# HuiyangYu/TGSFilter

Measured on AMD Instinct MI355X. Metric: filtered Gbases/sec (end-to-end, excl. gzip I/O), higher is better.
Workload: dtype u8

## Files before the change

### tgsfilter_amd/csrc/tgsf_emul_rt.h

```cpp
#pragma once
#include "tgsf_emul.h"
typedef void* rt_stream;
typedef void* rt_event;
static int rt_set_device(int) { return 0; }
static int rt_malloc(void** p, size_t n) { *p = calloc(n ? n : 1, 1); return *p ? 0 : 1; }
static void rt_free(void* p) { free(p); }
static void rt_host_free(void*) {}
static int rt_memset(void* p, int v, size_t n, rt_stream) { memset(p, v, n); return 0; }
static int rt_h2d(void* d, const void* s, size_t n, rt_stream) { memcpy(d, s, n); return 0; }
static int rt_d2h(void* d, const void* s, size_t n, rt_stream) { memcpy(d, s, n); return 0; }
static int rt_stream_create(rt_stream* s) { *s = nullptr; return 0; }
static void rt_stream_destroy(rt_stream) {}
static int rt_sync(rt_stream) { return 0; }
static int rt_device_sync() { return 0; }
static int rt_stream_wait(rt_stream, rt_event) { return 0; }
static int rt_event_create(rt_event* e) { *e = nullptr; return 0; }
static void rt_event_destroy(rt_event) {}
static int rt_event_record(rt_event, rt_stream) { return 0; }
static int rt_event_sync(rt_event) { return 0; }
static int rt_event_ms(float* ms, rt_event, rt_event) { *ms = 0.0f; return 0; }
static int rt_last_error() { return 0; }
static const char* rt_errstr(int) { return "emulation error"; }
template <class F>
static void emul_launch(unsigned grid, unsigned block, F f)
{
    using namespace tgsf_emul;
    gridDim = {grid, 1, 1}; blockDim = {block, 1, 1};
    const char* ord = getenv("TGSF_EMUL_ORDER");
    const bool reverse = ord && !strcmp(ord, "reverse");
    for (unsigned b0 = 0; b0 < grid; b0++)
        for (unsigned t0 = 0; t0 < block; t0++) {
            const unsigned b = reverse ? grid - 1 - b0 : b0, t = reverse ? block - 1 - t0 : t0;
            blockIdx = {b, 0, 0}; threadIdx = {t, 0, 0}; f();
        }
}
#define TGSF_LAUNCH(kernel, grid, block, stream, ...) ((void)(stream), emul_launch((grid), (block), [&] { kernel(__VA_ARGS__); }))
#define TGSF_LAUNCH_COOP(kernel, grid, block, stream, ...) ((void)(stream), emul_launch((grid), 1u, [&] { kernel(__VA_ARGS__); }))
static unsigned grid_cap(unsigned g) { return g > 8u ? 8u : g; }
```

### tgsfilter_amd/csrc/tgsf_lib.hip

```cpp
#include <algorithm>
#include <type_traits>

#include "tgsf_kernels.h"
constexpr size_t kErrorCap = 512;
#include "tgsf_rt.h"
#if defined(TGSF_EMUL)
namespace tgsf_emul { thread_local Dim3 threadIdx, blockIdx, blockDim, gridDim; }
#endif

using namespace tgsf;

static const char* knob(const char* name)
{
    static const bool on = [] { const char* e = getenv("TGSF_DEBUG_KNOBS"); return e && e[0] == '1'; }();
    return on ? getenv(name) : nullptr;
}

struct tgsf_ctx : rt_ctx {
    tgsf_params params;
    std::vector<std::string> adapters;
    DevParams P;
    DevBatch B;
    rt_stream stream;
    rt_stream last_stream;
    bool own_stream;
    uint64_t cap_bases, cap_chunks;
    uint32_t cap_reads, max_read_len, n_bins;
    static constexpr unsigned endtab_grid = 512;
    static constexpr unsigned stats_grid = 768;
    bool flat_scan = true;
    int suffix_filter = 2;
    bool no_hot32 = false;
    uint64_t ctr_words;
    int scratch_cols;
    uint8_t *d_seq, *d_qual;
    uint64_t* d_off;
    uint64_t* d_qoff;
    uint32_t* d_lenin;
    tgsf_read_result* d_out_reads;
    tgsf_fragment* d_out_frags;
    uint32_t* d_out_nfrags;
    bool profile;
    float stage_ms[TGSF_N_STAGES];
    uint32_t prof_batches;
    static constexpr int kProfRing = 64;
    rt_event ev[kProfRing][TGSF_N_STAGES + 1];
    rt_event ev_aux[kProfRing][3];
    int prof_pending;
    rt_stream aux;
    rt_event ev_fork, ev_join;
    uint32_t* h_pinned = nullptr;
    static constexpr size_t kStageBytes = 32u << 20;
    uint8_t* stage[2] = {nullptr, nullptr};
    rt_event stage_ev[2] = {nullptr, nullptr};
    uint32_t h_words_[8];
    uint32_t* h_status;
    uint32_t* pend_nf_p;
    tgsf_batch_out* pend_out = nullptr;
    struct Pending { tgsf_batch_in in; tgsf_read_result* reads; tgsf_fragment* frags; uint32_t fcap; uint32_t* nfrags; rt_stream st; };
    Pending pending[TGSF_MAX_ENQUEUED];
    uint32_t n_pending = 0;
    uint32_t* ovf_ring = nullptr;
    uint32_t* bp_ring = nullptr;
    uint32_t h_ovf[TGSF_MAX_ENQUEUED];
    uint32_t pool_regrown = 0;
};

static const int kMaxLenParam = 1 << 28;
static void adapter_rules(const tgsf_params& p, DevParams& P)
{
    P.max_nw = 1;
    P.min_Q = 1 << 30;
    for (int a = 0; a < p.n_adapters; a++) {
        const int Q = p.adapter_len[a];
        P.Q[a] = Q;
        if (Q > 64 && P.max_nw < 2) P.max_nw = 2;
        if (Q > 128 && P.max_nw < 4) P.max_nw = 4;
        if (Q > 256) P.max_nw = kWideNW;
        if (Q < P.min_Q) P.min_Q = Q;
        int km = Q - p.mid_match_len + 1;
        int ke = Q - p.end_match_len + 1;
        P.k_mid[a] = km > Q - 1 ? Q - 1 : km;
        P.k_end[a] = ke > Q - 1 ? Q - 1 : ke;
        const float w = (float)Q / p.end_sim;
        P.w5[a] = p.end_len + (w < (float)kMaxLenParam ? (int)w : kMaxLenParam);
        P.need_end[a] = P.need_mid[a] = Q + 1;
        for (int m = Q; m >= 0; m--) {
            if (m >= p.end_match_len && (float)m / (float)Q >= p.end_sim) P.need_end[a] = m;
            if (m >= p.mid_match_len && (float)m / (float)Q >= p.mid_sim) P.need_mid[a] = m;
        }
    }
}

static void fill_peq(const std::vector<std::string>& adapters, size_t slots, int W, std::vector<uint64_t>& fwd, std::vector<uint64_t>& rev)
{
    const size_t per_ad = (size_t)256 * W;
    fwd.assign(slots * per_ad, 0);
    rev.assign(slots * per_ad, 0);
    for (size_t a = 0; a < adapters.size(); a++) {
        const std::string& s = adapters[a];
        const int Q = (int)s.size();
        for (int r = 0; r < Q && r < 64 * W; r++) {
            const uint8_t cf = (uint8_t)s[r], cr = (uint8_t)s[Q - 1 - r];
            fwd[a * per_ad + (size_t)cf * W + (r >> 6)] |= 1ull << (r & 63);
            rev[a * per_ad + (size_t)cr * W + (r >> 6)] |= 1ull << (r & 63);
        }
    }
}

static int build_tables(tgsf_ctx* c)
{
    DevParams& P = c->P;
    const int A = c->params.n_adapters;
    std::vector<uint8_t> ad((size_t)kMaxAdapters * kMaxQ, 0);
    std::vector<uint64_t> fwd, rev, top((size_t)kMaxAdapters * 256, 0);
    fill_peq(c->adapters, kMaxAdapters, kPeqW, fwd, rev);
    for (int a = 0; a < A; a++) {
        const int Q = P.Q[a];
        memcpy(&ad[(size_t)a * kMaxQ], c->adapters[a].data(), (size_t)Q);
        if (Q <= 64) {
            const int sh = 64 - Q;
            const uint64_t pad = sh ? ((1ull << sh) - 1ull) : 0ull;
            for (int sym = 0; sym < 256; sym++)
                top[(size_t)a * 256 + sym] = (fwd[((size_t)a * 256 + sym) * kPeqW] << sh) | pad;
        }
    }
    uint8_t* d_ad; uint64_t *d_f, *d_r, *d_t;
    int e;
    if ((e = dev_alloc(c, &d_ad, ad.size()))) return e;
    if ((e = dev_alloc(c, &d_f, fwd.size()))) return e;
    if ((e = dev_alloc(c, &d_r, rev.size()))) return e;
    if ((e = dev_alloc(c, &d_t, top.size()))) return e;
    rt_h2d(d_ad, ad.data(), ad.size(), c->stream);
    rt_h2d(d_f, fwd.data(), fwd.size() * 8, c->stream);
    rt_h2d(d_r, rev.data(), rev.size() * 8, c->stream);
    rt_h2d(d_t, top.data(), top.size() * 8, c->stream);
    rt_sync(c->stream);
    P.adapter = d_ad; P.peq_fwd = d_f; P.peq_rev = d_r; P.peq_top = d_t;
    P.peq_fwd_w = P.peq_rev_w = nullptr;
    if (P.max_nw > 4) {
        fill_peq(c->adapters, (size_t)A, kWideNW, fwd, rev);
        uint64_t *d_fw, *d_rw;
        if ((e = dev_alloc(c, &d_fw, fwd.size()))) return e;
        if ((e = dev_alloc(c, &d_rw, rev.size()))) return e;
        rt_h2d(d_fw, fwd.data(), fwd.size() * 8, c->stream);
        rt_h2d(d_rw, rev.data(), rev.size() * 8, c->stream);
        rt_sync(c->stream);
        P.peq_fwd_w = d_fw; P.peq_rev_w = d_rw;
    }
    return 0;
}

extern "C" int tgsf_abi_version(void) { return TGSF_ABI_VERSION; }
extern "C" const char* tgsf_backend(void) { return kTgsfEmul ? "emulation" : "hip:gfx950"; }

#if !defined(TGSF_EMUL)
__global__ void k_noop(int* p) { if (p) *p = 0; }
static void set_wait_mode(int device)
{
    const char* e = getenv("TGSF_SYNC");
    if (!e || strcmp(e, "blocking") != 0) return;
    if (hipSetDevice(device) == hipSuccess) { (void)hipSetDeviceFlags(hipDeviceScheduleBlockingSync); (void)hipGetLastError(); }
}
#endif
extern "C" int tgsf_prepare_device(int device)
{
#if !defined(TGSF_EMUL)
    int ndev = 0;
    if (hipGetDeviceCount(&ndev) != hipSuccess || device < 0 || device >= ndev) return TGSF_E_NO_DEVICE;
    set_wait_mode(device);
    if (hipSetDevice(device) != hipSuccess) return TGSF_E_HIP;
    hipLaunchKernelGGL(k_noop, dim3(1), dim3(64), 0, 0, (int*)nullptr);
    if (hipDeviceSynchronize() != hipSuccess) return TGSF_E_HIP;
    {
        static const char a0[] = "GTTTTCGCATTTATCGTGAAACGCTTTCGCGTTTTTCGTGCGCCGCTTCA";
        static const char a1[] = "TGAAGCGGCGCACGAAAAACGCGAAAGCGTTTCACGATAAATGCGAAAAC";
        tgsf_params p;
        memset(&p, 0, sizeof p);
        p.struct_size = sizeof p;
        p.min_len = 100; p.max_len = 2147483647; p.min_q = 0; p.max_q = 255; p.bc_len = 150;
        p.end_len = 150; p.end_match_len = 4; p.mid_match_len = 35; p.extra_len = 50;
        p.end_sim = 0.75f; p.mid_sim = 0.9f; p.filter = 1; p.qtype = 33; p.kmer = 11;
        p.n_adapters = 2; p.adapters[0] = a0; p.adapters[1] = a1; p.adapter_len[0] = p.adapter_len[1] = 50;
        p.max_batch_bases = 1 << 16; p.max_batch_reads = 16; p.max_read_len = 1 << 14;
        tgsf_ctx* c = nullptr;
        if (tgsf_create(&p, device, &c) == TGSF_OK) {
            std::vector<uint8_t> seq(8192), qual(8192, (uint8_t)'5');
            for (size_t i = 0; i < seq.size(); i++) seq[i] = "ACGT"[(i * 2654435761u >> 13) & 3];
            memcpy(&seq[4096 + 1000], a0, 50);
            const uint64_t off[2] = {0, 4096};
            const uint32_t len[2] = {3000, 4000};
            tgsf_read_result res[2];
            tgsf_fragment fr[64];
            tgsf_batch_in in;
            memset(&in, 0, sizeof in);
            in.seq = seq.data(); in.qual = qual.data(); in.offsets = off; in.lengths = len; in.n_reads = 2; in.n_bytes = seq.size();
            tgsf_batch_out out{res, fr, 64, 0};
            (void)tgsf_submit(c, &in, &out);
            tgsf_destroy(c);
        }
    }
#else
    (void)device;
#endif
    return TGSF_OK;
}

extern "C" int tgsf_device_location(int device, char* bus_id, int len, int* numa_node)
{
    if (numa_node) *numa_node = -1;
    if (bus_id && len > 0) bus_id[0] = 0;
#if !defined(TGSF_EMUL)
    int ndev = 0;
    if (hipGetDeviceCount(&ndev) != hipSuccess || device < 0 || device >= ndev) return TGSF_E_NO_DEVICE;
    char id[64] = {0};
    if (hipDeviceGetPCIBusId(id, (int)sizeof id, device) != hipSuccess) return TGSF_E_HIP;
    for (char* p = id; *p; p++) if (*p >= 'A' && *p <= 'F') *p = (char)(*p - 'A' + 'a');
    if (bus_id && len > 0) { strncpy(bus_id, id, (size_t)len - 1); bus_id[len - 1] = 0; }
    if (numa_node) {
        const std::string path = std::string("/sys/bus/pci/devices/") + id + "/numa_node";
        if (FILE* f = fopen(path.c_str(), "r")) {
            int v = -1;
            if (fscanf(f, "%d", &v) == 1) *numa_node = v;
            fclose(f);
        }
    }
    return TGSF_OK;
#else
    if (bus_id && len > 0) snprintf(bus_id, (size_t)len, "emul:%d", device);
    if (numa_node)
        if (const char* e = knob("TGSF_EMUL_NUMA")) {
            int k = 0;
            for (const char* c = e; *c; k++) {
                if (k == device) { *numa_node = atoi(c); break; }
                while (*c && *c != ',') c++;
                if (*c == ',') c++;
            }
        }
    return TGSF_OK;
#endif
}

extern "C" const char* tgsf_last_error(tgsf_ctx* ctx) { return ctx ? ctx->error.c_str() : g_create_error.c_str(); }

extern "C" void tgsf_destroy(tgsf_ctx* c)
{
    if (!c) return;
    if (c->B.bp_allowed && c->B.bp_state && knob("TGSF_TRACE_BP")) {
        uint32_t w[4] = {0, 0, 0, 0};
        uint64_t pl[4] = {0, 0, 0, 0};
        uint32_t sg[4] = {0, 0, 0, 0};
        if (!rt_d2h(w, c->B.bp_state, sizeof w, c->stream) && !rt_d2h(pl, c->B.plan, sizeof pl, c->stream) && !rt_d2h(sg, c->B.seg_info, sizeof sg, c->stream) && !rt_sync(c->stream))
            fprintf(stderr, "tgsf: clean tables as a by-product of the raw pass: %u batches speculated; the next would%s; the last batch: %llu bases a direct clean pass scans, "
                            "%llu bases its own did, %u work items in that pass\n", w[1], w[0] ? "" : " not", (unsigned long long)pl[2], (unsigned long long)pl[3], sg[2]);
    }
    if (c->stream) { (void)rt_set_device(c->device); (void)rt_sync(c->stream); }
    for (int k = 0; k < tgsf_ctx::kProfRing; k++) {
        for (rt_event e : c->ev[k]) rt_event_destroy(e);
        for (rt_event e : c->ev_aux[k]) rt_event_destroy(e);
    }
    if (c->h_pinned) rt_host_free(c->h_pinned);
    for (int i = 0; i < 2; i++) {
        if (c->stage[i]) rt_host_free(c->stage[i]);
        rt_event_destroy(c->stage_ev[i]);
    }
    rt_event_destroy(c->ev_fork);
    rt_event_destroy(c->ev_join);
    if (c->aux) rt_stream_destroy(c->aux);
    if (c->own_stream && c->stream) rt_stream_destroy(c->stream);
    dev_free_all(c);
    delete c;
}

static int check_params(const tgsf_params* p)
{
    if (p->struct_size != sizeof(tgsf_params))
        return fail(nullptr, TGSF_E_INVALID, "tgsf_params.struct_size %u != %zu (ABI mismatch)", p->struct_size, sizeof(tgsf_params));
    if (p->n_adapters < 0 || p->n_adapters > TGSF_MAX_ADAPTERS)
        return fail(nullptr, TGSF_E_INVALID, "n_adapters %d outside [0,%d]", p->n_adapters, TGSF_MAX_ADAPTERS);
    if (p->min_repeat > 0 && (p->kmer < 1 || p->kmer > 32))
        return fail(nullptr, TGSF_E_UNSUPPORTED, "kmer (-k) %d: the repeat gate supports k-mer sizes 1..32 (the reference's k-mers are 64 bits)", p->kmer);
    if (p->min_len < 0) return fail(nullptr, TGSF_E_INVALID, "min_len (-l) %d: must be >= 0", p->min_len);
    if (p->end_len > kMaxLenParam) return fail(nullptr, TGSF_E_INVALID, "end_len (-E) %d: must be <= 2^28", p->end_len);
    if (p->extra_len > kMaxLenParam) return fail(nullptr, TGSF_E_INVALID, "extra_len (-T) %d: must be <= 2^28", p->extra_len);
    if (p->qtype != 33 && p->qtype != 64) return fail(nullptr, TGSF_E_INVALID, "qtype must be 33 or 64");
    if (p->bc_len < 0 || p->bc_len > kMaxBcLenTotal) return fail(nullptr, TGSF_E_INVALID, "bc_len (-e) outside [0,%d]", kMaxBcLenTotal);
    if (p->filter && p->n_adapters > 0) {
        if (!(p->end_sim > 0.f)) return fail(nullptr, TGSF_E_INVALID, "end_sim must be > 0");
        if (!(p->mid_sim > 0.f)) return fail(nullptr, TGSF_E_INVALID, "mid_sim must be > 0");
        if (p->end_len < 0) return fail(nullptr, TGSF_E_INVALID, "end_len must be >= 0");
        if (p->extra_len < 0) return fail(nullptr, TGSF_E_INVALID, "extra_len must be >= 0");
        if (p->end_match_len < 1) return fail(nullptr, TGSF_E_INVALID, "end_match_len must be >= 1");
        if (p->mid_match_len < 1) return fail(nullptr, TGSF_E_INVALID, "mid_match_len must be >= 1");
    }
    for (int a = 0; a < p->n_adapters; a++) {
        if (!p->adapters[a] || p->adapter_len[a] < 1 || p->adapter_len[a] > TGSF_MAX_ADAPTER_LEN)
            return fail(nullptr, TGSF_E_UNSUPPORTED, "adapter %d: length %d outside [1,%d]", a, p->adapter_len[a], TGSF_MAX_ADAPTER_LEN);
    }
    if (!p->max_batch_bases) return fail(nullptr, TGSF_E_INVALID, "max_batch_bases must be set");
    if (!p->max_batch_reads) return fail(nullptr, TGSF_E_INVALID, "max_batch_reads must be set");
    if (!p->max_read_len) return fail(nullptr, TGSF_E_INVALID, "max_read_len must be set");
    if (p->max_read_len > (1u << 28)) return fail(nullptr, TGSF_E_INVALID, "max_read_len above 2^28");
    return TGSF_OK;
}

struct Sizing {
    DevBatch B;
    uint64_t cap_bytes, cap_chunks;
    size_t nitems, scratch_waves;
    int scratch_cols, seg_cols, suffix_filter;
    bool flat_scan, no_hot32;
};

static Sizing size_context(const tgsf_params& p, const DevParams& P)
{
    Sizing S;
    DevBatch& B = S.B;
    memset(&B, 0, sizeof B);
    S.seg_cols = kSegCols; S.no_hot32 = false; S.flat_scan = true; S.suffix_filter = 2;
    if (const char* e = knob("TGSF_NO_HOT32")) S.no_hot32 = atoi(e) > 0;
    if (const char* e = knob("TGSF_SEG_COLS")) { int v = atoi(e); if (v >= 256 && v <= 65536) S.seg_cols = v & ~15; }
    if (const char* e = knob("TGSF_MID_FLAT")) S.flat_scan = atoi(e) > 0;
    if (const char* e = knob("TGSF_MID_FILTER")) { int v = atoi(e); if (v >= 0 && v <= 2) S.suffix_filter = v; }
    B.flat_pmax = 256; B.flat_pmin = 16; B.flat_f0 = 224;
    if (const char* e = knob("TGSF_FLAT_PMIN")) { int v = atoi(e); if (v >= 1 && v <= (1 << 20)) B.flat_pmin = (uint32_t)v; }
    if (const char* e = knob("TGSF_FLAT_PMAX")) { int v = atoi(e); if (v >= 1 && v <= (1 << 20)) B.flat_pmax = (uint32_t)v; }
    if (const char* e = knob("TGSF_FLAT_F0")) { int v = atoi(e); if (v >= 0 && v <= 256) B.flat_f0 = (uint32_t)v; }
    B.flat_pmin = 1u << flat_log2(B.flat_pmin); B.flat_pmax = 1u << flat_log2(B.flat_pmax);
    if (B.flat_pmax < B.flat_pmin) B.flat_pmax = B.flat_pmin;
    const uint64_t cap_bases = p.max_batch_bases;
    const size_t n = p.max_batch_reads;
    const int A = p.n_adapters > 0 ? p.n_adapters : 1;
    S.cap_bytes = cap_bases + 16ull * n + 64;
    const int min_len = p.min_len > 0 ? p.min_len : 1;
    uint64_t fcap64 = p.filter ? (cap_bases / (uint64_t)min_len + 16) : (uint64_t)n + 16;
    if (fcap64 > cap_bases + 16) fcap64 = cap_bases + 16;
    if (fcap64 < n + 16 && !p.filter) fcap64 = n + 16;
    B.fcap = (uint32_t)std::min<uint64_t>(fcap64, 0x7FFFFFF0ull);
    B.max_tiles = (p.max_read_len + kTileBases - 1) / kTileBases;
    uint64_t pool = cap_bases / 64 + 65536 + (uint64_t)n * 16u * (uint64_t)A;
    B.pool_cap = (uint32_t)std::min<uint64_t>(pool, 1ull << 28);
    if (const char* e = knob("TGSF_POOL_CAP")) { const long long v = atoll(e); if (v >= 1 && v < (1ll << 28)) B.pool_cap = (uint32_t)v; }
    S.nitems = n + (size_t)B.fcap;
    S.cap_chunks = cap_bases / 16u + 2ull * n;
    if (S.cap_chunks >= 0xFFFFFFF0ull) S.flat_scan = false;
    if (S.cap_chunks >= (1ull << 30) || !S.flat_scan) S.suffix_filter = 0;
    bool any = false;
    for (int a = 0; a < p.n_adapters; a++) any |= P.Q[a] > 32 && P.Q[a] <= 64 && P.k_mid[a] >= 0 && P.k_mid[a] <= kSuffixMaxK;
    if (!any || !p.filter) S.suffix_filter = 0;
    if (S.suffix_filter) {
        B.rc_cap = (uint32_t)std::min<uint64_t>(S.cap_chunks / 25u + 4096u, 1ull << 24);
        if (const char* e = knob("TGSF_RECHECK_CAP")) { int v = atoi(e); if (v >= 0) B.rc_cap = (uint32_t)v; }
    }
    B.rep_long_cap = (uint32_t)std::min<uint64_t>((cap_bases + 16ull * n) / kRepShare + 16, (uint64_t)B.fcap + 16);
    if (p.min_repeat > 0 && p.kmer >= 12 && p.kmer <= 31) {
        B.rep_tab_log2 = 4;
        while (B.rep_tab_log2 < 40 && (1ull << B.rep_tab_log2) < 2ull * p.max_read_len) B.rep_tab_log2++;
        B.rep_max_plog = kRepMaxPlog;
        if (const char* e = knob("TGSF_REP_MAX_PLOG")) { int v = atoi(e); if (v >= 0 && v <= 20) B.rep_max_plog = (uint32_t)v; }
    }
    B.work_cap = (uint32_t)std::min<uint64_t>(2 * (cap_bases / kTileBases) + S.nitems + 16, 0x7FFFFFF0ull);
    B.clean_force = p.only_qc ? 1u : 0u;
    B.bp_allowed = (p.filter && !p.only_qc && (p.head_trim > 0 || p.tail_trim > 0) &&
                    p.head_trim >= 0 && p.tail_trim >= 0) ? 1u : 0u;
    static_assert(kTileBases < (1 << 13), "staged bytes of a tile fit the work list's 13 bits");
    if (const char* f = knob("TGSF_CLEAN_TABLES")) {
        if (!strcmp(f, "direct")) { B.clean_force = 1; B.bp_allowed = 0; }
        else if (!strcmp(f, "difference") && !p.only_qc) { B.clean_force = 2; B.bp_allowed = 0; }
        else if (!strcmp(f, "byproduct") && B.bp_allowed) B.clean_force = 3;
    }
    int maxcols = 1;
    for (int a = 0; a < p.n_adapters; a++) {
        int kmax = std::max(std::max(P.k_end[a], P.k_mid[a]), 0);
        maxcols = std::max(maxcols, P.Q[a] + std::min(P.Q[a], kmax) + 1);
    }
    S.scratch_cols = maxcols;
    int col_words = P.max_nw;
    if (P.max_nw > 4) { col_words = 1; for (int a = 0; a < p.n_adapters; a++) col_words = std::max(col_words, (P.Q[a] + 63) / 64); }
    size_t lane_words = (size_t)(maxcols + 1) * 2 * (size_t)col_words;
    if (P.max_nw > 4) lane_words = std::min<size_t>(lane_words, (1u << 17) + 2 * (size_t)col_words) + 4 * (size_t)col_words + 64;
    B.scratch_wave_words = lane_words * 64;
    B.scratch_mid_wave0 = ((size_t)n * A * 2 + 63) / 64 + 1;
    S.scratch_waves = B.scratch_mid_wave0 + ((size_t)n * A + 63) / 64 + 1;
    return S;
}

static int bring_up(tgsf_ctx* c)
{
    c->h_status = c->h_words_; c->pend_nf_p = c->h_words_ + 4;
#if !defined(TGSF_EMUL)
    int ndev = 0;
    hipError_t he = hipGetDeviceCount(&ndev);
    if (he != hipSuccess || ndev <= 0)
        return fail(nullptr, TGSF_E_NO_DEVICE, "no HIP device available (%s); libtgsf has no CPU fallback", hipGetErrorString(he));
    if (c->device < 0 || c->device >= ndev) return fail(nullptr, TGSF_E_NO_DEVICE, "device %d out of range (%d devices)", c->device, ndev);
    set_wait_mode(c->device);
    if ((he = hipSetDevice(c->device)) != hipSuccess) return fail(nullptr, TGSF_E_HIP, "hipSetDevice: %s", hipGetErrorString(he));
    if ((he = hipStreamCreateWithFlags(&c->stream, hipStreamNonBlocking)) != hipSuccess) return fail(nullptr, TGSF_E_HIP, "hipStreamCreate: %s", hipGetErrorString(he));
    c->own_stream = true;
    uint32_t* pw = nullptr;
    if (hipHostMalloc((void**)&pw, 64, hipHostMallocDefault) == hipSuccess && pw) {
        memset(pw, 0, 64);
        c->h_pinned = pw; c->h_status = pw; c->pend_nf_p = pw + 4;
    }
    int lo = 0, hi = 0;
    (void)hipDeviceGetStreamPriorityRange(&lo, &hi);
    he = hipStreamCreateWithPriority(&c->aux, hipStreamNonBlocking, hi);
    if (he != hipSuccess ||
        (he = hipEventCreateWithFlags(&c->ev_fork, hipEventDisableTiming)) != hipSuccess ||
        (he = hipEventCreateWithFlags(&c->ev_join, hipEventDisableTiming)) != hipSuccess)
        return fail(nullptr, TGSF_E_HIP, "auxiliary stream: %s", hipGetErrorString(he));
    if (c->params.max_batch_bases > (8u << 20)) {
        for (int i = 0; i < 2; i++)
            if (hipHostMalloc((void**)&c->stage[i], tgsf_ctx::kStageBytes, hipHostMallocDefault) != hipSuccess ||
                hipEventCreateWithFlags(&c->stage_ev[i], hipEventDisableTiming) != hipSuccess)
                return fail(nullptr, TGSF_E_HIP, "pinned staging buffers: allocation failed");
    }
#endif
    c->last_stream = c->stream;
    return TGSF_OK;
}

static int allocate(tgsf_ctx* c, const Sizing& S)
{
    DevBatch& B = c->B;
    const size_t n = c->cap_reads;
    const int A = std::max(c->params.n_adapters, 1);
    const size_t tiles = 2 * ((size_t)B.max_tiles + 2);
    int e = 0;
    if (!e) e = dev_alloc(c, &c->d_seq, S.cap_bytes);
    if (!e) e = dev_alloc(c, &c->d_qual, S.cap_bytes);
    if (!e) e = dev_alloc(c, &c->d_off, n + 1);
    if (!e) e = dev_alloc(c, &c->d_qoff, n + 1);
    if (!e) e = dev_alloc(c, &c->d_lenin, n);
    if (!e) e = dev_alloc(c, &B.len, n);
    if (!e) e = dev_alloc(c, &B.sumq, n);
    if (!e) e = dev_alloc(c, &B.flags, n);
    if (!e) e = dev_alloc(c, &B.clip5, n * A);
    if (!e) e = dev_alloc(c, &B.clip3, n * A);
    if (!e) e = dev_alloc(c, &B.mid_head, n);
    if (!e) e = dev_alloc(c, &B.mid_best, n * A);
    if (!e) e = dev_alloc(c, &B.mid_cnt, n);
    if (!e) e = dev_alloc(c, &B.mid_gate, n * A);
    if (!e) e = dev_alloc(c, &B.pool, (size_t)B.pool_cap);
    if (!e) e = dev_alloc(c, &B.pool_n, 4);
    if (!e) e = dev_alloc(c, &B.seg_cnt, n + 1);
    if (!e) e = dev_alloc(c, &B.chk_cnt, n + 1);
    if (c->suffix_filter) {
        if (!e) e = dev_alloc(c, &B.chk_mark, (size_t)4 * (size_t)(S.cap_chunks / 32u + 8u));
        if (!e) e = dev_alloc(c, &B.rc_list, (size_t)B.rc_cap + 1);
        if (!e) e = dev_alloc(c, &B.rc_n, 4);
    }
    if (!e) e = dev_alloc(c, &B.nfr, n + 1);
    if (!e) e = dev_alloc(c, &B.scan_part, n / kScanTile + 2);
    if (!e) e = dev_alloc(c, &B.trimmed, n);
    if (!e) e = dev_alloc(c, &B.rep_next, 2 + (size_t)B.rep_long_cap);
    if (B.rep_tab_log2) {
        if (!e) e = dev_alloc(c, &B.rep_tab, (size_t)1 << B.rep_tab_log2);
        if (!e) e = dev_alloc(c, &B.rep_lock, 4);
        if (!e) rt_memset(B.rep_lock, 0, 16, c->stream);
    }
    if (!e) e = dev_alloc(c, &B.tile_hist, tiles);
    if (!e) e = dev_alloc(c, &B.tile_cnt, tiles);
    if (!e) e = dev_alloc(c, &B.tile_base, tiles);
    if (!e) e = dev_alloc(c, &B.tile_fill, tiles);
    if (!e) e = dev_alloc(c, &B.seg_info, 4);
    if (!e) e = dev_alloc(c, &B.perm, S.nitems);
    if (!e) e = dev_alloc(c, &B.work, 2 * (size_t)B.work_cap);
    if (!e) e = dev_alloc(c, &B.frag_off, (size_t)B.fcap);
    if (!e) e = dev_alloc(c, &B.frag_qoff, (size_t)B.fcap);
    if (!e) e = dev_alloc(c, &B.frag_len, (size_t)B.fcap);
    if (!e) e = dev_alloc(c, &B.frag_sum, (size_t)B.fcap);
    if (!e) e = dev_alloc(c, &B.frag_read, (size_t)B.fcap);
    if (!e) e = dev_alloc(c, &B.frag_start, (size_t)B.fcap);
    if (!e) e = dev_alloc(c, &B.frag_flags, (size_t)B.fcap);
    if (!e) e = dev_alloc(c, &B.raw_tab, 2 * (size_t)c->n_bins * 5);
    if (!e) e = dev_alloc(c, &B.whole, n);
    if (!e) e = dev_alloc(c, &B.plan, 4);
    if (B.bp_allowed) {
        if (!e) e = dev_alloc(c, &B.spec, n);
        if (!e) e = dev_alloc(c, &B.spec_sum, n);
        if (!e) e = dev_alloc(c, &B.bp_state, 4);
        if (!e) e = dev_alloc(c, &c->bp_ring, TGSF_MAX_ENQUEUED);
    }
    if (!e) e = dev_alloc(c, &B.scratch, S.scratch_waves * B.scratch_wave_words);
    if (!e) e = dev_alloc(c, &B.ctr, (size_t)c->ctr_words);
    if (!e) e = dev_alloc(c, &B.status, 4);
    if (!e) e = dev_alloc(c, &c->ovf_ring, TGSF_MAX_ENQUEUED);
    if (!e) e = dev_alloc(c, &c->d_out_reads, n);
    if (!e) e = dev_alloc(c, &c->d_out_frags, (size_t)B.fcap);
    if (!e) e = dev_alloc(c, &c->d_out_nfrags, 4);
    if (e) return e;
    rt_memset(B.ctr, 0, c->ctr_words * 8, c->stream);
    rt_memset(B.status, 0, 16, c->stream);
    rt_memset(c->ovf_ring, 0, TGSF_MAX_ENQUEUED * 4, c->stream);
    B.ovf = c->ovf_ring;
    if (B.bp_allowed) {
        const uint32_t init[4] = {1u, 0u, 0u, 0u};
        rt_memset(c->bp_ring, 0, TGSF_MAX_ENQUEUED * 4, c->stream);
        (void)rt_h2d(B.bp_state, init, sizeof init, c->stream);
        B.bp_used = c->bp_ring;
    }
    rt_memset(B.raw_tab, 0, 2 * (size_t)c->n_bins * 5 * 8, c->stream);
    rt_sync(c->stream);
    return TGSF_OK;
}

extern "C" int tgsf_create(const tgsf_params* p, int device, tgsf_ctx** out)
{
    if (!p || !out) return fail(nullptr, TGSF_E_INVALID, "null argument");
    *out = nullptr;
    int e = check_params(p);
    if (e) return e;
    tgsf_ctx* c = new tgsf_ctx();
    c->alloc_slack = 64;
    c->params = *p;
    c->device = device;
    for (int a = 0; a < p->n_adapters; a++) {
        c->adapters.emplace_back(p->adapters[a], (size_t)p->adapter_len[a]);
        c->params.adapters[a] = c->adapters.back().data();
    }
    DevParams& P = c->P;
    P.min_len = p->min_len; P.max_len = p->max_len; P.min_q = p->min_q; P.max_q = p->max_q;
    P.bc_len = p->bc_len; P.head_trim = p->head_trim; P.tail_trim = p->tail_trim; P.end_len = p->end_len;
    P.end_match_len = p->end_match_len; P.mid_match_len = p->mid_match_len; P.extra_len = p->extra_len;
    P.end_sim = p->end_sim; P.mid_sim = p->mid_sim; P.discard = p->discard; P.filter = p->filter;
    P.only_qc = p->only_qc; P.qtype = p->qtype; P.n_adapters = p->n_adapters;
    P.no_qual = p->no_qual ? 1 : 0;
    P.min_repeat = p->min_repeat; P.kmer = p->kmer;
    c->cap_bases = p->max_batch_bases;
    c->cap_reads = p->max_batch_reads;
    c->max_read_len = p->max_read_len;
    c->n_bins = tgsf_n_bins(p->max_read_len);
    P.n_bins = c->n_bins;
    c->ctr_words = tgsf_ctr_len(p->bc_len, c->n_bins);
    adapter_rules(*p, P);
    const Sizing S = size_context(*p, P);
    c->B = S.B; c->cap_chunks = S.cap_chunks; c->scratch_cols = S.scratch_cols; P.seg_cols = S.seg_cols;
    c->flat_scan = S.flat_scan; c->suffix_filter = S.suffix_filter; c->no_hot32 = S.no_hot32;

    if ((e = bring_up(c)) || (e = build_tables(c)) || (e = allocate(c, S))) {
        if (!c->error.empty()) g_create_error = c->error;
        tgsf_destroy(c);
        return e;
    }
    *out = c;
    return TGSF_OK;
}

static const char* kStageNames[TGSF_N_STAGES] = {
    "prepare+sort", "stats_raw", "gate_reads", "end_tables_raw", "end_windows", "mid_scan",
    "mid_resolve", "regions", "repeat_gate", "stats_clean", "gate_frags+end_tables_clean", "finalize"};

extern "C" const char* tgsf_stage_name(int s) { return (s >= 0 && s < TGSF_N_STAGES) ? kStageNames[s] : ""; }

static unsigned blocks_for(uint64_t n, unsigned block) { return (unsigned)std::max<uint64_t>(1, (n + block - 1) / block); }

static int harvest_profile(tgsf_ctx* c, rt_stream st)
{
    if (!c->prof_pending) return TGSF_OK;
    const int he = rt_sync(st);
    if (he) return fail(c, TGSF_E_HIP, "stream synchronize failed: %s", rt_errstr(he));
    (void)rt_sync(c->aux);
    for (int k = 0; k < c->prof_pending; k++)
        for (int i = 0; i < TGSF_N_STAGES; i++) {
            float ms = 0.f;
            const int e = (i == 3 || i == 4) ? rt_event_ms(&ms, c->ev_aux[k][i - 3], c->ev_aux[k][i - 2])
                                             : rt_event_ms(&ms, c->ev[k][i], c->ev[k][i + 1]);
            if (!e) c->stage_ms[i] += ms;
        }
    c->prof_pending = 0;
    return TGSF_OK;
}

template <int V> using int_c = std::integral_constant<int, V>;

template <class F>
static void with_width(int max_nw, F&& f)
{
    if (max_nw > 4) f(int_c<kWideNW>());
    else if (max_nw > 2) f(int_c<4>());
    else f(int_c<2>());
}

template <int MAXNA, class F>
static void with_adapters(int na, F&& f)
{
    static_assert(MAXNA == 2 || MAXNA == 4, "a pass takes up to two or up to four adapters");
    if (na == 1) return f(int_c<1>());
    if constexpr (MAXNA == 4) {
        if (na == 3) return f(int_c<3>());
        if (na != 2) return f(int_c<4>());
    }
    f(int_c<2>());
}

static void scan_u32(const DevBatch& B, uint32_t* a, uint32_t n, rt_stream st, uint32_t* part = nullptr)
{
    if (!part) part = B.scan_part;
    const unsigned nb = (n + kScanTile - 1) / kScanTile;
    TGSF_LAUNCH_COOP(k_scan_tiles, nb, 256, st, a, n, part);
    TGSF_LAUNCH_COOP(k_scan_top, 1, 64, st, part, (uint32_t)nb, a + n);
    TGSF_LAUNCH_COOP(k_scan_add, nb, 256, st, a, n, (const uint32_t*)part);
}

static int drain_pending(tgsf_ctx* c, bool implicit = false);

struct Run {
    tgsf_ctx* c;
    const tgsf_batch_in* in;
    DevBatch B;
    rt_stream st, ax;
    bool redo, profile;
    rt_event *evs, *evx;
    int stage, A;
    uint32_t n;
    unsigned gsmall, gstats, gfold, gwork, gfr;
    size_t tl;
    bool flat;
    unsigned gflat, gseg;
    uint64_t flat_chunks, max_segs;
};
static constexpr unsigned kBlock = 256;
static_assert(kMidThreads == kBlock, "k_mid_flat / k_mid_scan1 are launched with kBlock lanes a workgroup");

static void stage_mark(Run& r)
{
    if (r.profile) (void)rt_event_record(r.evs[r.stage], r.st);
    r.stage++;
}

static void stage_prepare(Run& r)
{
    const DevParams& P = r.c->P; const DevBatch& B = r.B; const rt_stream st = r.st;
    rt_memset(B.ovf, 0, 4, st);
    rt_memset(B.tile_hist, 0, r.tl, st);
    rt_memset(B.tile_fill, 0, r.tl, st);
    rt_memset(B.pool_n, 0, 4, st);
    rt_memset(B.plan, 0, 32, st);
    TGSF_LAUNCH(k_prepare, r.gsmall, kBlock, st, P, B, r.c->max_read_len);
    TGSF_LAUNCH_COOP(k_tile_scan, 1, 64, st, B, B.bp_allowed ? 2u : 1u);
    TGSF_LAUNCH(k_tile_scatter<false>, r.gsmall, kBlock, st, P, B);
    TGSF_LAUNCH(k_build_work<false>, r.gwork, kBlock, st, P, B);
}

static void stage_raw_stats(Run& r)
{
    const DevParams& P = r.c->P; const DevBatch& B = r.B; const rt_stream st = r.st;
    if (B.bp_allowed) {
        TGSF_LAUNCH((k_stats<false, true, true>), r.gstats, 64 * kStatsWaves, st, P, B);
        if (P.tail_trim > 0) TGSF_LAUNCH(k_tail_fix, grid_cap(std::min(blocks_for(r.n, 1024), 128u)), 1024, st, P, B);
    } else TGSF_LAUNCH((k_stats<false, true>), r.gstats, 64 * kStatsWaves, st, P, B);
    if (!r.redo) TGSF_LAUNCH(k_fold_raw<false>, r.gfold, kBlock, st, P, B);
}

static void stage_fork_ends(Run& r)
{
    tgsf_ctx* c = r.c;
    const DevParams& P = c->P; const DevBatch& B = r.B; const rt_stream ax = r.ax;
    (void)rt_event_record(c->ev_fork, r.st);
    (void)rt_stream_wait(ax, c->ev_fork);
    if (r.profile) (void)rt_event_record(r.evx[0], ax);
    for (uint32_t slab = 0; !r.redo && slab * (uint32_t)kMaxBcLen < (uint32_t)P.bc_len; slab++)
        TGSF_LAUNCH(k_end_tables<false>, grid_cap(c->endtab_grid), 64 * kEndWaves, ax, P, B, slab);
    if (r.profile) (void)rt_event_record(r.evx[1], ax);
    if (P.filter && r.A > 0)
        with_width(P.max_nw, [&](auto nw) { TGSF_LAUNCH(k_end_windows<decltype(nw)::value>, blocks_for((uint64_t)r.n * r.A * 2, 64), 64, ax, P, B); });
    if (r.profile) (void)rt_event_record(r.evx[2], ax);
    (void)rt_event_record(c->ev_join, ax);
}

static void launch_scans(Run& r, uint32_t mode)
{
    tgsf_ctx* c = r.c;
    const DevParams& P = c->P; const rt_stream ms = r.st;
    const int A = r.A;
    DevBatch Bm = r.B;
    Bm.mid_mode = mode;
    int a = 0;
    while (a < A) {
        if (P.Q[a] > 256) { TGSF_LAUNCH(k_mid_scanw<BvW>, r.gseg, kBlock, ms, P, Bm, a); a++; continue; }
        if (P.Q[a] > 192) { TGSF_LAUNCH(k_mid_scanw<Bv<4>>, r.gseg, kBlock, ms, P, Bm, a); a++; continue; }
        if (P.Q[a] > 128) { TGSF_LAUNCH(k_mid_scanw<Bv<3>>, r.gseg, kBlock, ms, P, Bm, a); a++; continue; }
        if (P.Q[a] > 64) { TGSF_LAUNCH(k_mid_scanw<Bv<2>>, r.gseg, kBlock, ms, P, Bm, a); a++; continue; }
        auto cls = [&](int x) {
            if (P.Q[x] <= 32 && !c->no_hot32) return 0;
            if (r.flat && mode == 0 && c->suffix_filter && P.Q[x] > 32 && P.k_mid[x] >= 0 && P.k_mid[x] <= kSuffixMaxK) return 2;
            return 1;
        };
        const int kind = cls(a);
        const bool narrow = kind == 0;
        const int width = narrow ? 2 : 4;
        int na = 0;
        while (a + na < A && na < width && P.Q[a + na] <= 64 && cls(a + na) == kind) na++;
        if (kind == 2) {
            Bm.mark_stride = (uint32_t)((r.flat_chunks / 32u + 7u) & ~3ull);
            rt_memset(Bm.chk_mark, 0, (size_t)na * Bm.mark_stride * 4u, ms);
            rt_memset(Bm.rc_n, 0, 4, ms);
            with_adapters<4>(na, [&](auto nc) {
                constexpr int NA = decltype(nc)::value;
                if (c->suffix_filter == 1) TGSF_LAUNCH((k_mid_flat<NA, Hot32, 1>), r.gflat, kBlock, ms, P, Bm, a, na);
                else TGSF_LAUNCH((k_mid_flat<NA, Hot32, 2>), r.gflat, kBlock, ms, P, Bm, a, na);
            });
            const unsigned grc = grid_cap(blocks_for(r.flat_chunks / 32u + 1u, (unsigned)kRecheckWords));
            TGSF_LAUNCH_COOP(k_mid_marks, grc, kBlock, ms, P, Bm, a, na);
            TGSF_LAUNCH(k_mid_recheck, grid_cap(2048u), kBlock, ms, P, Bm, a, na);
        } else if (r.flat && mode == 0) {
            if (narrow) with_adapters<2>(na, [&](auto nc) { constexpr int NA = decltype(nc)::value; TGSF_LAUNCH((k_mid_flat<NA, Hot32>), r.gflat, kBlock, ms, P, Bm, a, na); });
            else with_adapters<4>(na, [&](auto nc) { constexpr int NA = decltype(nc)::value; TGSF_LAUNCH((k_mid_flat<NA, Hot>), r.gflat, kBlock, ms, P, Bm, a, na); });
        } else {
            if (narrow) with_adapters<2>(na, [&](auto nc) { constexpr int NA = decltype(nc)::value; TGSF_LAUNCH((k_mid_scan1<NA, Hot32>), r.gseg, kBlock, ms, P, Bm, a, na); });
            else with_adapters<4>(na, [&](auto nc) { constexpr int NA = decltype(nc)::value; TGSF_LAUNCH((k_mid_scan1<NA, Hot>), r.gseg, kBlock, ms, P, Bm, a, na); });
        }
        a += na;
    }
}

static void launch_resolve(Run& r, const DevBatch& B)
{
    with_width(r.c->P.max_nw, [&](auto nw) { TGSF_LAUNCH(k_mid_resolve<decltype(nw)::value>, blocks_for((uint64_t)r.n * r.A, 64), 64, r.st, r.c->P, B); });
}

static void stage_mid_scan(Run& r)
{
    tgsf_ctx* c = r.c;
    const DevBatch& B = r.B;
    r.flat = c->flat_scan;
    r.gflat = 1;
    r.flat_chunks = 0;
    scan_u32(B, B.seg_cnt, r.n, r.st);
    if (r.flat) {
        scan_u32(B, B.chk_cnt, r.n, r.st);
        FlatSchedule S;
        r.flat_chunks = std::min<uint64_t>(r.in->n_bytes / 16u + (uint64_t)r.n, c->cap_chunks);
        flat_schedule((uint32_t)r.flat_chunks, B.flat_pmax, B.flat_pmin, B.flat_f0, S);
        r.gflat = grid_cap(blocks_for((uint64_t)S.d0[S.nph] + 128ull * (B.flat_pmax / B.flat_pmin) + 512u, kBlock));
    }
    r.max_segs = r.in->n_bytes / (uint64_t)c->P.seg_cols + 2ull * r.n + 1;
    r.gseg = blocks_for(r.max_segs, kBlock);
    launch_scans(r, 0);
}

static int replay_in_order(Run& r)
{
    tgsf_ctx* c = r.c;
    const DevParams& P = c->P; DevBatch& B = r.B; const rt_stream ms = r.st;
    const int A = r.A;
    const uint64_t cells = r.max_segs * (uint64_t)A + 1;
    if (cells > 0xFFFFFFF0ull) return fail(c, TGSF_E_CAPACITY, "middle scan: too many (segment, adapter) cells for the position-ordered pass");
    uint32_t *seg_n = nullptr, *part = nullptr;
    if (rt_malloc((void**)&seg_n, (size_t)(cells + 1) * 4 + 64) || rt_malloc((void**)&part, (size_t)(cells / kScanTile + 4) * 4 + 64)) {
        if (seg_n) rt_free(seg_n);
        return fail(c, TGSF_E_CAPACITY, "middle scan: no device memory for the position-ordered pass (%.1f GB)", (double)cells * 4e-9);
    }
    B.seg_n = seg_n;
    int rc = TGSF_OK;
    do {
        rt_memset(seg_n, 0, (size_t)(cells + 1) * 4, ms);
        TGSF_LAUNCH(k_mid_reset, r.gsmall, kBlock, ms, B, A);
        launch_scans(r, 1);
        scan_u32(B, seg_n, (uint32_t)cells, ms, part);
        uint32_t need = 0;
        int he = rt_d2h(&need, seg_n + cells, 4, ms);
        if (!he) he = rt_sync(ms);
        if (he) { rc = fail(c, TGSF_E_HIP, "middle scan (counting pass) failed: %s", rt_errstr(he)); break; }
        if (need > B.pool_cap) {
            const uint64_t want = (uint64_t)need + 1024;
            if (want > 0x7FFFFFF0ull) { rc = fail(c, TGSF_E_CAPACITY, "middle-adapter candidates: %u columns tie their reads' minima, more than one batch can list", need); break; }
            void* np = nullptr;
            if (rt_malloc(&np, (size_t)want * sizeof(MidCand) + 64)) {
                rc = fail(c, TGSF_E_CAPACITY, "middle-adapter candidates: no device memory for %llu slots (%.1f GB)", (unsigned long long)want, (double)want * sizeof(MidCand) * 1e-9);
                break;
            }
            for (void*& q : c->allocs) if (q == (void*)c->B.pool) q = np;
            rt_free(c->B.pool);
            c->B.pool = (MidCand*)np; c->B.pool_cap = (uint32_t)want;
            B.pool = c->B.pool; B.pool_cap = c->B.pool_cap;
            c->pool_regrown++;
        }
        if (knob("TGSF_TRACE_POOL"))
            fprintf(stderr, "tgsf: candidate pool overflow (or a read with a long candidate list): %u columns at their reads' minima, pool of %u slots%s; scanning again in position order\n", need, B.pool_cap,
                    c->pool_regrown ? " (grown)" : "");
        rt_memset(B.ovf, 0, 4, ms);
        launch_scans(r, 2);
        TGSF_LAUNCH(k_mid_link, r.gsmall, kBlock, ms, B, A);
        DevBatch Bm = B;
        Bm.mid_mode = 2;
        launch_resolve(r, Bm);
        const unsigned geach = grid_cap(std::min(blocks_for(need, 64), 65536u));
        if (need) with_width(P.max_nw, [&](auto nw) { TGSF_LAUNCH(k_mid_resolve_each<decltype(nw)::value>, geach, 64, ms, P, Bm); });
        he = rt_sync(ms);
        if (he) rc = fail(c, TGSF_E_HIP, "middle scan (position-ordered pass) failed: %s", rt_errstr(he));
    } while (0);
    rt_free(seg_n);
    rt_free(part);
    B.seg_n = nullptr;
    return rc;
}

static void stage_regions(Run& r)
{
    const DevParams& P = r.c->P; const DevBatch& B = r.B; const rt_stream st = r.st;
    (void)rt_stream_wait(st, r.c->ev_join);
    TGSF_LAUNCH(k_regions<false>, r.gsmall, kBlock, st, P, B);
    scan_u32(B, B.nfr, r.n, st);
    TGSF_LAUNCH(k_regions<true>, r.gsmall, kBlock, st, P, B);
}

static void stage_repeat_gate(Run& r)
{
    const DevParams& P = r.c->P; const DevBatch& B = r.B; const rt_stream st = r.st;
    rt_memset(B.rep_next, 0, 2 * sizeof(uint32_t), st);
    if (P.kmer < 12) TGSF_LAUNCH(k_repeat, grid_cap(256u), kRepThreads, st, P, B);
    else {
        TGSF_LAUNCH(k_repeat_long, r.gsmall, kBlock, st, P, B);
        if (P.kmer <= 15) TGSF_LAUNCH(k_repeat_keys<false>, grid_cap(256u), kRepThreads, st, P, B);
        else TGSF_LAUNCH(k_repeat_keys<true>, grid_cap(256u), kRepThreads, st, P, B);
    }
}

static void stage_clean_stats(Run& r)
{
    const DevParams& P = r.c->P; const DevBatch& B = r.B; const rt_stream st = r.st;
    rt_memset(B.tile_hist, 0, r.tl, st);
    rt_memset(B.tile_fill, 0, r.tl, st);
    const unsigned gfr = r.gfr;
    TGSF_LAUNCH(k_clean_plan, r.gsmall, kBlock, st, P, B);
    if (B.bp_allowed && !r.redo) TGSF_LAUNCH(k_clean_plan_next, 1, 64, st, B);
    TGSF_LAUNCH(k_fold_raw<true>, r.gfold, kBlock, st, P, B);
    TGSF_LAUNCH(k_frag_prepare, gfr, kBlock, st, P, B);
    TGSF_LAUNCH_COOP(k_tile_scan, 1, 64, st, B, 2u);
    TGSF_LAUNCH(k_tile_scatter<true>, gfr, kBlock, st, P, B);
    TGSF_LAUNCH(k_build_work<true>, r.gwork, kBlock, st, P, B);
    TGSF_LAUNCH((k_stats<true, true>), r.gstats, 64 * kStatsWaves, st, P, B);
}

static void stage_clean_tables(Run& r)
{
    const DevParams& P = r.c->P; const DevBatch& B = r.B; const rt_stream st = r.st;
    TGSF_LAUNCH(k_gate_frags, r.gfr, kBlock, st, P, B);
    for (uint32_t slab = 0; slab * (uint32_t)kMaxBcLen < (uint32_t)P.bc_len; slab++)
        TGSF_LAUNCH(k_end_tables<true>, grid_cap(r.c->endtab_grid), 64 * kEndWaves, st, P, B, slab);
}

static int run_pipeline(tgsf_ctx* c, const tgsf_batch_in* in, tgsf_read_result* d_reads, tgsf_fragment* d_frags,
                        uint32_t out_fcap, uint32_t* d_nfrags, rt_stream st, bool redo = false, uint32_t slot = 0)
{
    if (!redo) {
        if (c->n_pending == TGSF_MAX_ENQUEUED) { int e = drain_pending(c, true); if (e) return e; }
        slot = c->n_pending++;
        tgsf_ctx::Pending& pd = c->pending[slot];
        pd.in = *in; pd.reads = d_reads; pd.frags = d_frags; pd.fcap = out_fcap; pd.nfrags = d_nfrags; pd.st = st;
    }
    const DevParams& P = c->P;
    Run r;
    r.c = c; r.in = in; r.st = st; r.ax = c->aux; r.redo = redo;
    r.profile = c->profile && !redo && !kTgsfEmul;
    DevBatch& B = r.B = c->B;
    B.ovf = c->ovf_ring + slot;
    B.bp_used = c->bp_ring + slot;
    B.replay = redo ? 1u : 0u;
    B.seq = in->seq; B.qual = in->qual; B.off = in->offsets; B.len_in = in->lengths;
    B.qoff = in->qual_offsets ? in->qual_offsets : in->offsets;
    B.n = in->n_reads; B.n_bytes = in->n_bytes;
    const uint32_t n = r.n = B.n;
    r.A = P.n_adapters;
    c->last_stream = st;
    r.gsmall = grid_cap(std::min(blocks_for(n, kBlock), 2048u));
    r.gstats = grid_cap(c->stats_grid);
    r.tl = 2 * ((size_t)B.max_tiles + 2) * 4;
    r.gfold = grid_cap(std::min(blocks_for((uint64_t)P.n_bins * 5, kBlock), 1024u));
    r.gwork = grid_cap(std::min(blocks_for(in->n_bytes / kTileBases + n + 1, kBlock), 4096u));
    r.gfr = grid_cap(std::min(blocks_for((uint64_t)B.fcap + n, kBlock), 2048u));
    r.stage = 0;
    if (r.profile && c->prof_pending == tgsf_ctx::kProfRing) { int e = harvest_profile(c, st); if (e) return e; }
    r.evs = c->ev[r.profile ? c->prof_pending : 0];
    r.evx = c->ev_aux[r.profile ? c->prof_pending : 0];
    if (r.profile) {
        for (int i = 0; i <= TGSF_N_STAGES; i++) if (!r.evs[i]) (void)rt_event_create(&r.evs[i]);
        for (int i = 0; i < 3; i++) if (!r.evx[i]) (void)rt_event_create(&r.evx[i]);
    }
    const bool scan = P.filter && r.A > 0;

    stage_mark(r);
    stage_prepare(r);
    stage_mark(r);
    stage_raw_stats(r);
    stage_mark(r);
    TGSF_LAUNCH(k_gate_reads, r.gsmall, kBlock, st, P, B);
    stage_mark(r);
    stage_fork_ends(r);
    stage_mark(r);
    stage_mark(r);
    if (scan) {
        stage_mid_scan(r);
        if (redo) { int e = replay_in_order(r); if (e) return e; }
    }
    stage_mark(r);
    if (scan && !redo) launch_resolve(r, B);
    stage_mark(r);
    stage_regions(r);
    stage_mark(r);
    if (P.min_repeat > 0 && !P.only_qc) stage_repeat_gate(r);
    stage_mark(r);
    stage_clean_stats(r);
    stage_mark(r);
    stage_clean_tables(r);
    stage_mark(r);
    TGSF_LAUNCH(k_finalize, r.gsmall, kBlock, st, B, d_reads, d_frags, out_fcap, d_nfrags);
    stage_mark(r);
    const int he = rt_last_error();
    if (he) return fail(c, TGSF_E_HIP, "kernel launch failed: %s", rt_errstr(he));
    if (r.profile) { c->prof_batches++; c->prof_pending++; }
    return TGSF_OK;
}

static int text_h2d(tgsf_ctx* c, uint8_t* dst, const uint8_t* src, uint64_t n, rt_stream st)
{
#if !defined(TGSF_EMUL)
    hipPointerAttribute_t at;
    const bool known = hipPointerGetAttributes(&at, src) == hipSuccess && at.type != hipMemoryTypeUnregistered;
    (void)hipGetLastError();
    if (!known && c->stage[0] && n > (1u << 20)) {
        int he = 0, k = 0;
        for (uint64_t o = 0; o < n; o += tgsf_ctx::kStageBytes, k ^= 1) {
            const size_t m = (size_t)std::min<uint64_t>(tgsf_ctx::kStageBytes, n - o);
            (void)hipEventSynchronize(c->stage_ev[k]);
            memcpy(c->stage[k], src + o, m);
            he |= (int)hipMemcpyAsync(dst + o, c->stage[k], m, hipMemcpyHostToDevice, st);
            he |= (int)hipEventRecord(c->stage_ev[k], st);
        }
        return he;
    }
#endif
    (void)c;
    return rt_h2d(dst, src, n, st);
}

static int check_batch(tgsf_ctx* c, const tgsf_batch_in* in)
{
    if (!in || !in->seq || (!in->qual && !c->P.no_qual) || !in->offsets) return fail(c, TGSF_E_INVALID, "null batch pointer");
    if (in->n_reads == 0) return fail(c, TGSF_E_INVALID, "empty batch");
    if (in->n_reads > c->cap_reads) return fail(c, TGSF_E_CAPACITY, "batch has %u reads, context was sized for %u", in->n_reads, c->cap_reads);
    if (in->qual_offsets && !in->lengths) return fail(c, TGSF_E_INVALID, "qual_offsets requires explicit lengths");
    return TGSF_OK;
}

static int check_status(tgsf_ctx* c)
{
    const uint32_t code = c->h_status[0], detail = c->h_status[1];
    if (!code) return TGSF_OK;
    rt_memset(c->B.status, 0, 16, c->stream);
    rt_sync(c->stream);
    switch (code) {
    case DS_BAD_LEN: return fail(c, TGSF_E_DATA, "read %u: length 0 or above max_read_len %u", detail, c->max_read_len);
    case DS_TOO_MANY_REGIONS: return fail(c, TGSF_E_CAPACITY, "read %u has more than %d disjoint drop regions", detail, kMaxRegions);
    case DS_FRAG_CAP: return fail(c, TGSF_E_CAPACITY, "fragment capacity exceeded (%u)", detail);
    case DS_BAD_MEANQ: return fail(c, TGSF_E_DATA, "read %u: mean quality outside [0,256)", detail);
    default: return fail(c, TGSF_E_HIP, "device status %u", code);
    }
}

static int finish_pending(tgsf_ctx* c)
{
    tgsf_batch_out* out = c->pend_out;
    if (!out) return TGSF_OK;
    c->pend_out = nullptr;
    const uint32_t nf = *c->pend_nf_p;
    out->n_frags = nf;
    if (nf > out->frag_capacity || (nf && !out->frags))
        return fail(c, TGSF_E_CAPACITY, "batch produced %u fragments, caller provided room for %u", nf, out->frag_capacity);
    if (nf) {
        int he = rt_d2h(out->frags, c->d_out_frags, (size_t)nf * sizeof(tgsf_fragment), c->stream);
        if (!he) he = rt_sync(c->stream);
        if (he) return fail(c, TGSF_E_HIP, "device to host copy failed");
    }
    return TGSF_OK;
}

static int drain_pending(tgsf_ctx* c, bool implicit)
{
    int e = 0;
    const uint32_t np = c->n_pending;
    (void)rt_set_device(c->device);
    if (implicit) e = rt_device_sync();
    for (uint32_t i = 0; i < np && !e && !implicit; i++) {
        bool seen = c->pending[i].st == c->stream;
        for (uint32_t j = 0; j < i && !seen; j++) seen = c->pending[j].st == c->pending[i].st;
        if (!seen) e = rt_sync(c->pending[i].st);
    }
    if (!e) e = rt_sync(c->aux);
    if (!e) e = rt_d2h(c->h_status, c->B.status, 16, c->stream);
    if (!e && np) e = rt_d2h(c->h_ovf, c->ovf_ring, (size_t)np * 4, c->stream);
    if (!e) e = rt_sync(c->stream);
    c->n_pending = 0;
    if (e) { c->pend_out = nullptr; return fail(c, TGSF_E_HIP, "stream synchronize failed: %s", rt_errstr(e)); }
    e = check_status(c);
    if (e) { c->pend_out = nullptr; return e; }
    for (uint32_t i = 0; i < np; i++) {
        if (!c->h_ovf[i]) continue;
        if (implicit) {
            c->pend_out = nullptr;
            return fail(c, TGSF_E_INVALID, "batch %u of the %u enqueued since the last tgsf_wait has to be run again from its inputs (its middle-adapter candidates "
                                           "outgrew the pool) and only tgsf_wait may do that: call tgsf_wait at least every TGSF_MAX_ENQUEUED (%d) batches", i, np, TGSF_MAX_ENQUEUED);
        }
        const tgsf_ctx::Pending pd = c->pending[i];
        e = run_pipeline(c, &pd.in, pd.reads, pd.frags, pd.fcap, pd.nfrags, pd.st, true, i);
        if (!e && c->pend_out && pd.reads == c->d_out_reads) {
            int he = rt_d2h(c->pend_nf_p, c->d_out_nfrags, 4, pd.st);
            he |= rt_d2h(c->pend_out->reads, c->d_out_reads, (size_t)pd.in.n_reads * sizeof(tgsf_read_result), pd.st);
            if (he) e = fail(c, TGSF_E_HIP, "device to host copy failed");
        }
        uint32_t again = 0;
        if (!e) {
            int he = rt_d2h(c->h_status, c->B.status, 16, pd.st);
            if (!he) he = rt_d2h(&again, c->ovf_ring + i, 4, pd.st);
            if (!he) he = rt_sync(pd.st);
            if (!he) he = rt_sync(c->aux);
            if (he) e = fail(c, TGSF_E_HIP, "stream synchronize failed: %s", rt_errstr(he));
        }
        if (!e) e = check_status(c);
        if (!e && again) e = fail(c, TGSF_E_HIP, "middle-adapter candidate pool overflowed again after it was sized to fit");
        if (e) { c->pend_out = nullptr; return e; }
    }
    return TGSF_OK;
}

extern "C" int tgsf_wait(tgsf_ctx* c)
{
    if (!c) return TGSF_E_INVALID;
    const int e = drain_pending(c);
    if (e) return e;
    return finish_pending(c);
}

extern "C" int tgsf_submit_device(tgsf_ctx* c, const tgsf_batch_in* in, tgsf_batch_out* out,
                                  uint32_t* d_n_frags, void* hip_stream)
{
    if (!c) return TGSF_E_INVALID;
    int e = check_batch(c, in);
    if (e) return e;
    if (!out || !out->reads) return fail(c, TGSF_E_INVALID, "null output");
    if (((uintptr_t)in->seq & 15u) || (!c->P.no_qual && ((uintptr_t)in->qual & 15u))) return fail(c, TGSF_E_INVALID, "seq/qual device pointers must be 16-byte aligned");
    if (!in->n_bytes) return fail(c, TGSF_E_INVALID, "n_bytes is 0: a device batch must state the bytes it spans");
    if (in->n_bytes > c->cap_bases + 16ull * c->cap_reads) return fail(c, TGSF_E_CAPACITY, "batch spans %llu bytes, context was sized for %llu bases", (unsigned long long)in->n_bytes, (unsigned long long)c->cap_bases);
    (void)rt_set_device(c->device);
    rt_stream st = hip_stream ? (rt_stream)hip_stream : c->stream;
    return run_pipeline(c, in, out->reads, out->frags, out->frags ? out->frag_capacity : 0u, d_n_frags, st);
}

extern "C" int tgsf_submit_async(tgsf_ctx* c, const tgsf_batch_in* in, tgsf_batch_out* out)
{
    if (!c) return TGSF_E_INVALID;
    if (c->pend_out) return fail(c, TGSF_E_INVALID, "a batch is already pending on this context: call tgsf_wait first");
    int e = check_batch(c, in);
    if (e) return e;
    if (!out || !out->reads) return fail(c, TGSF_E_INVALID, "null output");
    const uint32_t n = in->n_reads;
    uint64_t span = in->n_bytes;
    if (!span) {
        span = in->lengths ? in->offsets[n - 1] + in->lengths[n - 1] : in->offsets[n];
        if (in->qual_offsets) span = std::max<uint64_t>(span, in->qual_offsets[n - 1] + in->lengths[n - 1]);
    }
    if (span > c->cap_bases + 16ull * c->cap_reads) return fail(c, TGSF_E_CAPACITY, "batch spans %llu bytes, context was sized for %llu bases", (unsigned long long)span, (unsigned long long)c->cap_bases);
    (void)rt_set_device(c->device);
    rt_stream st = c->stream;
    int he = 0;
    const bool one_buffer = in->qual == in->seq || c->P.no_qual;
    he |= text_h2d(c, c->d_seq, in->seq, span, st);
    if (!one_buffer) he |= text_h2d(c, c->d_qual, in->qual, span, st);
    he |= rt_h2d(c->d_off, in->offsets, (size_t)(in->lengths ? n : n + 1) * 8, st);
    if (in->lengths) he |= rt_h2d(c->d_lenin, in->lengths, (size_t)n * 4, st);
    if (in->qual_offsets) he |= rt_h2d(c->d_qoff, in->qual_offsets, (size_t)n * 8, st);
    if (he) return fail(c, TGSF_E_HIP, "host to device copy failed");
    tgsf_batch_in din = *in;
    din.seq = c->d_seq; din.qual = one_buffer ? c->d_seq : c->d_qual; din.offsets = c->d_off;
    din.lengths = in->lengths ? c->d_lenin : nullptr;
    din.qual_offsets = in->qual_offsets ? c->d_qoff : nullptr;
    din.n_bytes = span;
    e = run_pipeline(c, &din, c->d_out_reads, c->d_out_frags, c->B.fcap, c->d_out_nfrags, st);
    if (e) return e;
    *c->pend_nf_p = 0;
    he |= rt_d2h(c->pend_nf_p, c->d_out_nfrags, 4, st);
    he |= rt_d2h(out->reads, c->d_out_reads, (size_t)n * sizeof(tgsf_read_result), st);
    if (he) return fail(c, TGSF_E_HIP, "device to host copy failed");
    c->pend_out = out;
    return TGSF_OK;
}

extern "C" int tgsf_submit(tgsf_ctx* c, const tgsf_batch_in* in, tgsf_batch_out* out)
{
    const int e = tgsf_submit_async(c, in, out);
    return e ? e : tgsf_wait(c);
}

extern "C" int tgsf_counters_len(tgsf_ctx* c, uint64_t* n_words, int32_t* bc_len, uint32_t* n_bins)
{
    if (!c) return TGSF_E_INVALID;
    if (n_words) *n_words = c->ctr_words;
    if (bc_len) *bc_len = c->P.bc_len;
    if (n_bins) *n_bins = c->n_bins;
    return TGSF_OK;
}

extern "C" int tgsf_counters(tgsf_ctx* c, uint64_t* dst, uint64_t n_words)
{
    if (!c || !dst) return TGSF_E_INVALID;
    if (n_words < c->ctr_words) return fail(c, TGSF_E_CAPACITY, "counter buffer too small");
    int e = tgsf_wait(c);
    if (e) return e;
    int he = rt_d2h(dst, c->B.ctr, c->ctr_words * 8, c->stream);
    if (!he) he = rt_sync(c->stream);
    return he ? fail(c, TGSF_E_HIP, "device to host copy failed") : TGSF_OK;
}

extern "C" int tgsf_counters_used(tgsf_ctx* c, uint64_t* dst, uint64_t n_words, uint64_t rows[2])
{
    if (!c || !dst) return TGSF_E_INVALID;
    if (n_words < c->ctr_words) return fail(c, TGSF_E_CAPACITY, "counter buffer too small");
    int e = tgsf_wait(c);
    if (e) return e;
    const size_t head = tgsf_ctr_bin_table(0, c->P.bc_len, c->n_bins);
    int he = rt_d2h(dst, c->B.ctr, head * 8, c->stream);
    if (!he) he = rt_sync(c->stream);
    if (he) return fail(c, TGSF_E_HIP, "device to host copy failed");
    const uint64_t used[2] = {std::min<uint64_t>(dst[TGSF_CTR_ROWS], c->n_bins), std::min<uint64_t>(dst[TGSF_CTR_ROWS + 1], c->n_bins)};
    for (int b = 0; b < 4 && !he; b++) {
        const size_t at = tgsf_ctr_bin_table(b, c->P.bc_len, c->n_bins);
        const uint64_t r = used[b >> 1];
        if (r) he = rt_d2h(dst + at, c->B.ctr + at, (size_t)r * 5 * 8, c->stream);
    }
    if (!he) he = rt_sync(c->stream);
    if (rows) { rows[0] = used[0]; rows[1] = used[1]; }
    return he ? fail(c, TGSF_E_HIP, "device to host copy failed") : TGSF_OK;
}

extern "C" int tgsf_counters_merge(tgsf_ctx* dst, tgsf_ctx* src)
{
    if (!dst || !src || dst == src) return TGSF_E_INVALID;
    if (dst->ctr_words != src->ctr_words || dst->P.bc_len != src->P.bc_len || dst->device != src->device)
        return fail(dst, TGSF_E_INVALID, "tgsf_counters_merge: the contexts differ in tally layout or device");
    int e = tgsf_wait(src);
    if (e) return fail(dst, e, "%s", src->error.c_str());
    if ((e = tgsf_wait(dst))) return e;
    TGSF_LAUNCH(k_ctr_merge, grid_cap(blocks_for(dst->ctr_words, 256)), 256, dst->stream, dst->B.ctr, (const uint64_t*)src->B.ctr, dst->ctr_words);
    const int he = rt_sync(dst->stream);
    return he ? fail(dst, TGSF_E_HIP, "tgsf_counters_merge failed") : TGSF_OK;
}

extern "C" int tgsf_counters_device(tgsf_ctx* c, void** d_ptr, uint64_t* n_words)
{
    if (!c || !d_ptr) return TGSF_E_INVALID;
    *d_ptr = c->B.ctr;
    if (n_words) *n_words = c->ctr_words;
    return TGSF_OK;
}

extern "C" int tgsf_reset_counters(tgsf_ctx* c)
{
    if (!c) return TGSF_E_INVALID;
    int he = rt_memset(c->B.ctr, 0, c->ctr_words * 8, c->stream);
    if (!he) he = rt_memset(c->B.raw_tab, 0, 2 * (size_t)c->n_bins * 5 * 8, c->stream);
    if (!he) he = rt_sync(c->stream);
    return he ? fail(c, TGSF_E_HIP, "memset failed") : TGSF_OK;
}

extern "C" int tgsf_profile(tgsf_ctx* c, int enable)
{
    if (!c) return TGSF_E_INVALID;
    { int e = harvest_profile(c, c->last_stream); if (e) return e; }
    c->profile = enable != 0;
    memset(c->stage_ms, 0, sizeof c->stage_ms);
    c->prof_batches = 0;
    return TGSF_OK;
}

extern "C" int tgsf_stage_times(tgsf_ctx* c, float ms[TGSF_N_STAGES], uint32_t* n_batches)
{
    if (!c || !ms) return TGSF_E_INVALID;
    { int e = harvest_profile(c, c->last_stream); if (e) return e; }
    memcpy(ms, c->stage_ms, sizeof c->stage_ms);
    if (n_batches) *n_batches = c->prof_batches;
    return TGSF_OK;
}

extern "C" int tgsf_align_windows(tgsf_ctx* c, const uint8_t* seq, uint64_t n_bytes, const uint64_t* win_off,
                                  const uint32_t* win_len, const uint8_t* adapter_id, const int32_t* k, uint32_t n,
                                  int32_t* res, int32_t* ends)
{
    if (!c || !seq || !win_off || !win_len || !adapter_id || !k || !res || !ends) return TGSF_E_INVALID;
    if (!n) return TGSF_OK;
    for (uint32_t i = 0; i < n; i++) {
        if (adapter_id[i] >= c->P.n_adapters) return fail(c, TGSF_E_INVALID, "problem %u: adapter id out of range", i);
        if (win_len[i] == 0 || win_off[i] + win_len[i] > n_bytes) return fail(c, TGSF_E_INVALID, "problem %u: window outside the buffer", i);
        if (k[i] < 0) return fail(c, TGSF_E_INVALID, "problem %u: k < 0", i);
        const int Q = c->P.Q[adapter_id[i]];
        if (Q + std::min(Q, (int)k[i]) + 1 > c->scratch_cols)
            return fail(c, TGSF_E_CAPACITY, "problem %u: k larger than the context's thresholds allow for", i);
    }
    if ((size_t)n > (size_t)c->cap_reads * std::max(c->P.n_adapters, 1) * 2)
        return fail(c, TGSF_E_CAPACITY, "more alignment problems than the context was sized for");
    (void)rt_set_device(c->device);
    uint8_t *d_seq = nullptr, *d_aid = nullptr; uint64_t* d_off = nullptr; uint32_t* d_len = nullptr;
    int32_t *d_k = nullptr, *d_res = nullptr, *d_ends = nullptr;
    int e = 0;
    e |= rt_malloc((void**)&d_seq, n_bytes + 16);
    e |= rt_malloc((void**)&d_aid, n);
    e |= rt_malloc((void**)&d_off, (size_t)n * 8);
    e |= rt_malloc((void**)&d_len, (size_t)n * 4);
    e |= rt_malloc((void**)&d_k, (size_t)n * 4);
    e |= rt_malloc((void**)&d_res, (size_t)n * 16);
    e |= rt_malloc((void**)&d_ends, (size_t)n * 8);
    rt_stream st = c->stream;
    if (!e) {
        e |= rt_h2d(d_seq, seq, n_bytes, st);
        e |= rt_h2d(d_aid, adapter_id, n, st);
        e |= rt_h2d(d_off, win_off, (size_t)n * 8, st);
        e |= rt_h2d(d_len, win_len, (size_t)n * 4, st);
        e |= rt_h2d(d_k, k, (size_t)n * 4, st);
    }
    if (!e) {
        with_width(c->P.max_nw, [&](auto nw) {
            TGSF_LAUNCH(k_align_windows<decltype(nw)::value>, blocks_for(n, 64), 64, st, c->P, c->B, (const uint8_t*)d_seq, (const uint64_t*)d_off,
                        (const uint32_t*)d_len, (const uint8_t*)d_aid, (const int32_t*)d_k, n, d_res, d_ends);
        });
        e |= rt_d2h(res, d_res, (size_t)n * 16, st);
        e |= rt_d2h(ends, d_ends, (size_t)n * 8, st);
        e |= rt_sync(st);
    }
    rt_free(d_seq); rt_free(d_aid); rt_free(d_off); rt_free(d_len); rt_free(d_k); rt_free(d_res); rt_free(d_ends);
    return e ? fail(c, TGSF_E_HIP, "tgsf_align_windows: device operation failed") : TGSF_OK;
}
```

### tgsfilter_amd/csrc/tgsf_rt.h

```cpp
#pragma once
#include <stdarg.h>
#include <stdio.h>
#include <stdlib.h>
#include <string.h>

#include <string>
#include <vector>

#include "../../include/tgsf.h"

#if defined(TGSF_EMUL)
#include "tgsf_emul_rt.h"
#else
#include <hip/hip_runtime.h>
typedef hipStream_t rt_stream;
typedef hipEvent_t rt_event;
static int rt_set_device(int device) { return (int)hipSetDevice(device); }
static int rt_malloc(void** p, size_t n) { return (int)hipMalloc(p, n ? n : 1); }
static void rt_free(void* p) { (void)hipFree(p); }
static void rt_host_free(void* p) { (void)hipHostFree(p); }
static int rt_memset(void* p, int v, size_t n, rt_stream s) { return (int)hipMemsetAsync(p, v, n, s); }
static int rt_h2d(void* d, const void* s, size_t n, rt_stream st) { return (int)hipMemcpyAsync(d, s, n, hipMemcpyHostToDevice, st); }
static int rt_d2h(void* d, const void* s, size_t n, rt_stream st) { return (int)hipMemcpyAsync(d, s, n, hipMemcpyDeviceToHost, st); }
static int rt_stream_create(rt_stream* s) { return (int)hipStreamCreateWithFlags(s, hipStreamNonBlocking); }
static void rt_stream_destroy(rt_stream s) { (void)hipStreamDestroy(s); }
static int rt_sync(rt_stream s) { return (int)hipStreamSynchronize(s); }
static int rt_device_sync() { return (int)hipDeviceSynchronize(); }
static int rt_stream_wait(rt_stream s, rt_event e) { return (int)hipStreamWaitEvent(s, e, 0); }
static int rt_event_create(rt_event* e) { return (int)hipEventCreate(e); }
static void rt_event_destroy(rt_event e) { if (e) (void)hipEventDestroy(e); }
static int rt_event_record(rt_event e, rt_stream s) { return (int)hipEventRecord(e, s); }
static int rt_event_sync(rt_event e) { return (int)hipEventSynchronize(e); }
static int rt_event_ms(float* ms, rt_event a, rt_event b) { return (int)hipEventElapsedTime(ms, a, b); }
static int rt_last_error() { return (int)hipGetLastError(); }
static const char* rt_errstr(int e) { return hipGetErrorString((hipError_t)e); }
#define TGSF_LAUNCH(kernel, grid, block, stream, ...) hipLaunchKernelGGL(kernel, dim3(grid), dim3(block), 0, (stream), __VA_ARGS__)
#define TGSF_LAUNCH_COOP TGSF_LAUNCH
static unsigned grid_cap(unsigned g) { return g; }
#endif

struct rt_ctx {
    int device = 0;
    std::string error;
    std::vector<void*> allocs;
    size_t alloc_slack = 0;
};

static thread_local std::string g_create_error;

static int fail(rt_ctx* c, int code, const char* fmt, ...)
{
    char buf[kErrorCap];
    va_list ap;
    va_start(ap, fmt);
    vsnprintf(buf, sizeof buf, fmt, ap);
    va_end(ap);
    if (c) c->error = buf; else g_create_error = buf;
    return code;
}

template <class T>
static int dev_alloc(rt_ctx* c, T** p, size_t count)
{
    void* v = nullptr;
    int e = rt_malloc(&v, count * sizeof(T) + c->alloc_slack);
    if (e) return fail(c, TGSF_E_HIP, "device allocation of %zu bytes failed: %s", count * sizeof(T), rt_errstr(e));
    c->allocs.push_back(v);
    *p = (T*)v;
    return 0;
}

static void dev_free_all(rt_ctx* c) { for (void* p : c->allocs) rt_free(p); }
```

### tgsfilter_amd/host/prepass.cpp

```cpp
#include "prepass.h"
#include <chrono>
#include <cstdio>

#include <unistd.h>

#include <algorithm>
#include <cstdlib>
#include <cstring>
#include <iostream>
#include <thread>
#include <unordered_map>
#include <vector>

#include "api.h"
#include "fatal.h"

namespace host {

const char* const kAdapterLib[22] = {
    "ATCTCTCTCTTTTCCTCCTCCTCCGTTGTTGTTGTTGAGAGAGAT",
    "ATCTCTCTCAACAACAACAACGGAGGAGGAGGAAAAGAGAGAGAT",
    "AAAAAAAAAAAAAAAAAATTAACGGAGGAGGAGGA",
    "TCCTCCTCCTCCGTTAATTTTTTTTTTTTTTTTTT",
    "AATGTACTTCGTTCAGTTACGTATTGCT",
    "AGCAATACGTAACTGAACGAAGTACATT",
    "GCAATACGTAACTGAACGAAGT",
    "ACTTCGTTCAGTTACGTATTGC",
    "GTTTTCGCATTTATCGTGAAACGCTTTCGCGTTTTTCGTGCGCCGCTTCA",
    "TGAAGCGGCGCACGAAAAACGCGAAAGCGTTTCACGATAAATGCGAAAAC",
    "GGCGTCTGCTTGGGTGTTTAACCTTTTTGTCAGAGAGGTTCCAAGTCAGAGAGGTTCCT",
    "AGGAACCTCTCTGACTTGGAACCTCTCTGACAAAAAGGTTAAACACCCAAGCAGACGCC",
    "GGAACCTCTCTGACTTGGAACCTCTCTGACAAAAAGGTTAAACACCCAAGCAGACGCCAGCAAT",
    "ATTGCTGGCGTCTGCTTGGGTGTTTAACCTTTTTGTCAGAGAGGTTCCAAGTCAGAGAGGTTCC",
    "TTTTTTTTCCTGTACTTCGTTCAGTTACGTATTGCT",
    "AGCAATACGTAACTGAACGAAGTACAGGAAAAAAAA",
    "GCAATACGTAACTGAACGAAGTACAGG",
    "CCTGTACTTCGTTCAGTTACGTATTGC",
    "ACGTAACTGAACGAAGTACAGG",
    "CCTGTACTTCGTTCAGTTACGT",
    "CTTGCGGGCGGCGGACTCTCCTCTGAAGATAGAGCGACAGGCAAG",
    "CTTGCCTGTCGCTCTATCTTCAGAGGAGAGTCCGCCGCCCGCAAG",
};

std::string rev_comp(const std::string& s)
{
    static char comp[256];
    static bool init = false;
    if (!init) {
        memset(comp, 'N', sizeof comp);
        const char* a = "AGCTagctMRWSYKmrwsyk";
        const char* b = "TCGAtcgaKYWSRMkywsrm";
        for (int i = 0; a[i]; i++) comp[(unsigned char)a[i]] = b[i];
        init = true;
    }
    std::string r;
    r.reserve(s.size());
    for (size_t i = s.size(); i-- > 0;) r += comp[(unsigned char)s[i]];
    return r;
}

static int check_base_content(const std::vector<std::string>& ends, int check_len, int seq_num, float end_bias)
{
    static const struct Col { uint8_t of[256]; Col() { memset(of, 4, sizeof of); of['A'] = of['a'] = 0; of['T'] = of['t'] = 1; of['G'] = of['g'] = 2; of['C'] = of['c'] = 3; } } col;
    std::vector<int> cnt5((size_t)check_len * 5, 0);
    for (const std::string& s : ends) {
        const size_t n = std::min(s.size(), (size_t)check_len);
        for (size_t i = 0; i < n; i++) cnt5[i * 5 + col.of[(unsigned char)s[i]]]++;
    }
    std::vector<int> cnt((size_t)check_len * 4, 0);
    for (int i = 0; i < check_len; i++) for (int j = 0; j < 4; j++) cnt[(size_t)i * 4 + j] = cnt5[(size_t)i * 5 + j];
    const int max_diff = (int)((seq_num * end_bias) / 100);
    int trim = 0;
    for (int i = 1; i < check_len - 1; i++) {
        const int ld = std::min(i, 5), rd = std::min(check_len - i - 1, 5);
        bool left = false, right = false;
        for (int j = 0; j < 4; j++) {
            for (int x = 1; x <= ld; x++)
                if (abs(cnt[(size_t)i * 4 + j] - cnt[(size_t)(i - x) * 4 + j]) > max_diff) { left = true; break; }
            for (int x = 1; x <= rd; x++)
                if (abs(cnt[(size_t)(i + x) * 4 + j] - cnt[(size_t)i * 4 + j]) > max_diff) { right = true; break; }
        }
        if (left && right) trim = i + 1;
    }
    return trim;
}

static double pp_now() { return std::chrono::duration<double>(std::chrono::steady_clock::now().time_since_epoch()).count(); }
static double g_pp_create = 0, g_pp_align = 0; static int g_pp_calls = 0;

static void adapter_search(const Options& o, const std::vector<std::string>& ends, std::string& adapter, float& depth)
{
    adapter.clear(); depth = 0.f;
    float min_sim = o.mid_sim;
    if (min_sim < 0.9) min_sim = 0.9f;
    if (ends.empty()) return;

    tgsf_params p;
    memset(&p, 0, sizeof p);
    p.struct_size = sizeof p;
    p.min_len = 100; p.max_len = 2147483647; p.min_q = 0; p.max_q = 255; p.bc_len = 0;
    p.end_len = 0; p.extra_len = 0; p.end_sim = 0.75f; p.mid_sim = 0.9f; p.filter = 1; p.qtype = 33;
    p.n_adapters = 22;
    int k[22];
    size_t max_q = 0;
    for (int a = 0; a < 22; a++) {
        p.adapters[a] = kAdapterLib[a];
        p.adapter_len[a] = (int)strlen(kAdapterLib[a]);
        k[a] = (int)((1 - min_sim) * p.adapter_len[a]) + 1;
        max_q = std::max(max_q, (size_t)p.adapter_len[a]);
    }
    p.end_match_len = 2; p.mid_match_len = (int)max_q;
    const size_t per_call = 4096;
    p.max_batch_reads = (uint32_t)(per_call * 22 / (22 * 2) + 64);
    p.max_batch_bases = 1 << 20; p.max_read_len = 1 << 16;
    tgsf_ctx* ctx = nullptr;
    const double c0 = pp_now();
    if (lib().create(&p, o.devices.empty() ? o.device : o.devices[0], &ctx) != TGSF_OK) { std::cerr << "Error: " << lib().last_error(nullptr) << std::endl; quit(255); }

    g_pp_create += pp_now() - c0;
    std::unordered_map<int, int> maps;
    std::vector<uint8_t> buf; std::vector<uint64_t> off; std::vector<uint32_t> len; std::vector<uint8_t> aid;
    std::vector<int32_t> kk, res, eds;
    for (size_t b = 0; b < ends.size(); b += per_call) {
        const size_t e = std::min(ends.size(), b + per_call);
        buf.clear(); off.clear(); len.clear(); aid.clear(); kk.clear();
        for (size_t i = b; i < e; i++) {
            const uint64_t o0 = buf.size();
            buf.insert(buf.end(), ends[i].begin(), ends[i].end());
            if (ends[i].empty()) continue;
            for (int a = 0; a < 22; a++) { off.push_back(o0); len.push_back((uint32_t)ends[i].size()); aid.push_back((uint8_t)a); kk.push_back(k[a]); }
        }
        const uint32_t n = (uint32_t)off.size();
        if (!n) continue;
        res.assign((size_t)n * 4, 0); eds.assign((size_t)n * 2, 0);
        const double a0 = pp_now();
        if (lib().align_windows(ctx, buf.data(), buf.size(), off.data(), len.data(), aid.data(), kk.data(), n, res.data(), eds.data()) != TGSF_OK) {
            std::cerr << "Error: " << lib().last_error(ctx) << std::endl; quit(255);
        }
        g_pp_align += pp_now() - a0; g_pp_calls++;
        for (uint32_t i = 0; i < n; i++)
            if (res[(size_t)i * 4 + 1] > 0)
                maps[(int)aid[i]] += res[(size_t)i * 4 + 2] - res[(size_t)i * 4 + 0];
    }
    lib().destroy(ctx);
    std::vector<std::pair<int, int>> vec(maps.begin(), maps.end());
    std::sort(vec.begin(), vec.end(), [](const std::pair<int, int>& a, const std::pair<int, int>& b) { return a.second > b.second; });
    if (vec.empty()) return;
    const int best = vec.front().first;
    const std::string cand = kAdapterLib[best];
    const float mean_dep = (float)maps[best] / (float)cand.size();
    if (mean_dep >= 2 * min_sim) { adapter = cand; depth = mean_dep; }
}

PrepassResult run_prepass(Options& o, const std::function<bool(Rec&)>& next_record)
{
    PrepassResult R;
    const double t0 = pp_now();
    int check_len = std::max(std::max(o.end_len, o.bc_len), 100);
    int min_len = std::max(o.min_len, 2 * check_len);
    const int max_seq = std::max(o.ad_num, o.bc_num);
    std::vector<std::string> ends5, ends3;
    const bool need5 = o.filter && (o.head_trim < 0 || o.adapter_file.empty());
    const bool need3 = o.filter && (o.tail_trim < 0 || o.adapter_file.empty());
    int seq_num = 0, min_qc = 255, max_qc = 0;
    {
        Rec r;
        const bool has_qual = o.in_type != 0;
        while (next_record(r)) {
            const int L = (int)r.len;
            if (L < min_len) continue;
            if (seq_num >= max_seq) break;
            seq_num++;
            if (need5) ends5.emplace_back(r.seq, (size_t)check_len);
            if (need3) ends3.emplace_back(rev_comp(std::string(r.seq + (L - check_len), (size_t)check_len)));
            if (has_qual)
                for (int i = 0; i < check_len; i++) { const char c = r.qual[i]; if (min_qc > c) min_qc = c; if (max_qc < c) max_qc = c; }
        }
    }
    const double t_read = pp_now() - t0;
    if (o.in_type == 1 || o.in_type == 2) {
        if (min_qc >= 33 && min_qc <= 78 && max_qc >= 33 && max_qc <= 127) R.qtype = 33;
        else if (min_qc >= 64 && min_qc <= 108 && max_qc >= 64 && max_qc <= 127) R.qtype = 64;
        else R.qtype = min_qc < 55 ? 33 : 64;
        std::cerr << "INFO: base quality scoring: Phred" << R.qtype << std::endl;
        const int maxq = max_qc - R.qtype;
        if (o.min_q >= 0) {
            if (o.min_q >= maxq) {
                std::cerr << "Warning: max base quality score was: " << maxq << std::endl;
                std::cerr << "INFO: Please reset -q parameter." << std::endl;
                quit(255);
            }
        } else {
            if (maxq > 10 && o.read_type == "clr") o.min_q = 10;
            else if (maxq > 20 && o.read_type == "hifi") o.min_q = 20;
            else if (maxq > 10 && o.read_type == "ont") o.min_q = 10;
            else o.min_q = 0;
        }
    }
    const double t1 = pp_now();
    double t_bc = 0;
    if (o.filter) {
        {
            std::thread t3;
            if (o.tail_trim < 0) t3 = std::thread([&] { R.trim3p = check_base_content(ends3, check_len, seq_num, o.end_bias); });
            if (o.head_trim < 0) R.trim5p = check_base_content(ends5, check_len, seq_num, o.end_bias);
            if (t3.joinable()) t3.join();
        }
        if (o.head_trim < 0 && o.tail_trim < 0 && R.trim5p > o.bc_len) R.trim5p = o.bc_len;
        t_bc = pp_now() - t1;
        if (o.adapter_file.empty()) {
            adapter_search(o, ends5, R.adapter5p, R.depth5p);
            adapter_search(o, ends3, R.adapter3p, R.depth3p);
        }
    }
    if (getenv("TGSF_TIMING"))
        fprintf(stderr, "PREPASS: %d reads looked at in %.3f s | base content %.3f | adapter search %.3f (contexts %.3f, %d alignment calls %.3f)\n",
                seq_num, t_read, t_bc, pp_now() - t1 - t_bc, g_pp_create, g_pp_calls, g_pp_align);
    return R;
}

}
```

### tgsfilter_amd/host/prepass.h

```cpp
#pragma once
#include <functional>
#include <string>
#include <vector>

#include "fastx.h"
#include "options.h"

namespace host {

extern const char* const kAdapterLib[22];

std::string rev_comp(const std::string& s);

struct PrepassResult {
    int qtype = 0;
    int trim5p = 0, trim3p = 0;
    std::string adapter5p, adapter3p;
    float depth5p = 0.f, depth3p = 0.f;
};

PrepassResult run_prepass(Options& o, const std::function<bool(Rec&)>& next_record);

}
```

### tgsfilter_amd/host/run.h

```cpp
#pragma once
#include <memory>

#include "api.h"
#include "pipeline.h"
#include "prepass.h"
#include "report.h"
#include "shard.h"

namespace host {

int cpu_budget();
[[noreturn]] void leave(int code);
bool detached();

struct Run {
    explicit Run(Options& opts) : o(opts) {}

    int set_up_ranks();
    int check_file_types();
    void open_input();
    void open_output_early();
    void prepass();
    void make_contexts();
    void filter_pass();
    void downsample();
    void sum_tallies();
    void report();
    void timing_lines();

    Options& o;
    RankLink link;
    bool shard_may_use_rccl = false;
    bool sharded = false;
    bool timing = false;
    double t_epoch0 = 0, t_start = 0;
    double t_prepass = 0, t_pipe = 0, t_parse = 0, t_gpu = 0, t_write = 0, t_widle = 0, t_first = 0;

    std::string html;
    bool fasta_in = false;
    InputBytes in;
    bool streaming = false;
    size_t chunk_bytes = 64u << 20;
    int scan_threads = 1;
    size_t text_off = 0, text_size = 0;
    const char* text = nullptr;
    std::unique_ptr<RecordIndex> records_p;
    std::unique_ptr<ChunkReader> open_stream();

    std::string out_path;
    bool plain_file_out() const;
    MappedWriter mapped;
    Output out;
    bool fastq_out = false, run_filter_pass = true;

    PrepassResult pp;
    std::vector<std::string> adapters;

    uint64_t batch_text = 0;
    uint32_t batch_reads = 1u << 16;
    const Api* api = nullptr;
    double t_load = 0, t_dev = 0, t_libwait = 0;
    const RcclApi* R = nullptr;
    struct RcclUp { std::atomic<int> done{0}; int rc = TGSF_OK; std::string err; void* comm = nullptr; };
    std::shared_ptr<RcclUp> rccl_state = std::make_shared<RcclUp>();
    std::thread rccl_up;
    bool use_rccl = false;
    bool ranks_own_gpus = false;
    tgsf_params p;
    std::vector<int> ctx_dev;
    std::vector<tgsf_ctx*> ctxs;
    double t_p0 = 0;

    std::unique_ptr<Channel<std::shared_ptr<Batch>>> to_gpu, to_writer;
    std::vector<int> raw_lens, clean_lens;
    uint64_t raw_bases = 0, clean_bases = 0;
    uint64_t own_raw_bases = 0;
    std::vector<CleanRec> clean_recs;
    BatchStore store;
    std::atomic<uint64_t> stream_text{0};
    std::atomic<double> stream_share{0.0};
    std::mutex gpu_time_m;
    bool numa_bind = false;
    std::vector<int> dev_node;
    std::vector<double> dev_submit_s;
    std::vector<uint64_t> dev_bytes, dev_batches;
    int fill_threads = 1, populate_threads = 1;
    uint64_t fill_min = 1u << 20, stride_bytes = 2ull << 30;
    bool release_input = false, release_output = false;
    bool mapped_out = false;
    void reader_body();
    void feed(size_t k);
    void bind_to_node_of(size_t k);
    void writer_body();
    void fill_job(const std::shared_ptr<Batch>& b, size_t lo, size_t hi);
    void batch_done(std::shared_ptr<Batch> b);

    MappedWriter down_mapped;
    bool open_down_mapped(uint64_t capacity, uint64_t speculative);
    uint64_t down_bases = 0, down_job_recs = 0, down_job_bases = 0;
    std::vector<int> down_lens;
    std::vector<uint64_t> down_t;
    double t_dsel = 0, t_dcreate = 0, t_dqc = 0, t_dwrite = 0, t_dclose = 0, t_dsubmit = 0, t_dfirst = 0, d_kept = 0, d_span = 0;
    int n_dsubmit = 0;
    bool d_in_place = false, d_mapped = false;
    std::vector<char> select_kept();
    void second_pass(const std::vector<char>& keep);
    std::thread start_qc_feed(const std::vector<char>& keep, tgsf_ctx*& qctx, tgsf_ctx*& qctx2);
    void feed_in_place(const std::vector<uint32_t>& by_addr, const tgsf_params& qp, uint64_t kept_span, tgsf_ctx* qctx, tgsf_ctx*& qctx2);
    void feed_packed(const std::vector<char>& keep, const tgsf_params& qp, size_t room, tgsf_ctx* qctx);
    void write_kept(const std::vector<char>& keep);
    void merge_down_tallies(tgsf_ctx* qctx, tgsf_ctx* qctx2);

    uint64_t nw = 0;
    int32_t bc = 0;
    uint32_t nbins = 0;
    std::vector<uint64_t> t;
    double t_x0 = 0, t_rccl_wait = 0, t_allreduce = 0;
    int rccl_ranks = 0;
    std::string tally_route;
    bool reports() const { return !sharded || link.rank == 0; }
};

void add_tallies(std::vector<uint64_t>& v, const std::vector<uint64_t>& part, int32_t bc, uint32_t nbins);
std::vector<uint64_t> pack_rows(const std::vector<uint64_t>& v, int32_t bc, uint32_t nbins);
void add_rows(std::vector<uint64_t>& v, const std::vector<uint64_t>& ru, int32_t bc, uint32_t nbins);

}
```

### tgsfilter_amd/host/run_pipeline.cpp

```cpp
#include "run.h"

#include <sched.h>

namespace host {

void Run::reader_body()
{
    CpuScope cpu(CPU_BATCHER);
    if (!run_filter_pass) { for (size_t d = 0; d < ctxs.size(); d++) to_gpu->put(nullptr); return; }
    std::unique_ptr<RecordIndex::Cursor> rd;
    if (!streaming) rd.reset(new RecordIndex::Cursor(*records_p));
    std::unique_ptr<ChunkReader> cr;
    if (streaming) cr = open_stream();
    std::shared_ptr<Chunk> ch;
    size_t ch_at = 0;
    bool over = false;
    Rec r;
    auto fresh = [&] { return store.get(); };
    std::shared_ptr<Batch> b = fresh();
    const double t0 = now_s();
    double waited = 0;
    uint64_t next_id = 0;
    auto flush = [&] {
        if (b->recs.empty()) return;
        const double w0 = now_s();
        b->id = next_id++;
        to_gpu->put(std::move(b));
        waited += now_s() - w0;
        b = fresh();
    };
    auto next_record = [&]() {
        if (!streaming) return rd->next(r);
        while (!over && (!ch || ch_at >= ch->recs.size())) {
            flush();
            if (ch && !ch->message.empty()) std::cerr << ch->message << std::endl;
            if (ch && ch->last) { over = true; break; }
            ch = cr->next(o.in_file);
            ch_at = 0;
            if (!ch) { over = true; break; }
            stream_text.store(cr->text_bytes());
            stream_share.store(cr->consumed());
        }
        if (over) return false;
        r = ch->recs[ch_at++];
        return true;
    };
    auto bad_cut = [&](size_t at) {
        die("--ranks / --shard: the input cannot be cut near byte " + std::to_string(at) + " the way one sequential reader would read it "
            "(lines the reader skips, or a malformed record, near there): run it without --ranks / --shard");
    };
    const char* last_end = nullptr;
    while (next_record()) {
        const size_t L = r.len;
        if (L > p.max_read_len) die("read longer than the supported maximum");
        const char* rec_end = (fasta_in ? r.seq : r.qual) + L;
        if (sharded && !last_end && link.rank > 0 && r.name != text + 1) bad_cut(text_off);
        last_end = rec_end;
        if (!b->recs.empty() && ((uint64_t)(rec_end - b->base) > batch_text || b->recs.size() >= batch_reads)) flush();
        if (b->recs.empty()) { b->base = r.name; b->hold = ch; }
        b->off.push_back((uint64_t)(r.seq - b->base));
        b->qoff.push_back(fasta_in ? b->off.back() : (uint64_t)(r.qual - b->base));
        b->len.push_back((uint32_t)L); b->recs.push_back(r);
        b->span = (uint64_t)(rec_end - b->base);
        if (b->span > p.max_batch_bases) die("record larger than a batch");
        b->bases += L;
        raw_bases += L; raw_lens.push_back((int)L);
    }
    if (sharded && link.rank + 1 < link.world) {
        const char* e = last_end ? last_end : text;
        const char* const end = text + text_size;
        if (e < end && *e == '\r') e++;
        if (e < end && *e == '\n') e++;
        if (e != end || !records_p->end_message().empty()) bad_cut(text_off + text_size);
    }
    flush();
    for (size_t d = 0; d < ctxs.size(); d++) to_gpu->put(nullptr);
    t_parse = now_s() - t0 - waited;
    std::sort(raw_lens.begin(), raw_lens.end());
}

void Run::bind_to_node_of(size_t k)
{
    const Api& L = *api;
    int node = -1;
    char bus[64];
    if (L.device_location(ctx_dev[k], bus, (int)sizeof bus, &node) == TGSF_OK && node >= 0) {
        const char* sysfs = knob("TGSF_SYSFS_NODES");
        std::ifstream f(std::string(sysfs ? sysfs : "/sys/devices/system/node") + "/node" + std::to_string(node) + "/cpulist");
        std::string list;
        cpu_set_t set;
        CPU_ZERO(&set);
        int n_set = 0;
        if (f && std::getline(f, list)) {
            size_t i = 0;
            while (i < list.size()) {
                const int a = atoi(list.c_str() + i);
                int b = a;
                size_t j = list.find_first_of(",-", i);
                if (j != std::string::npos && list[j] == '-') { b = atoi(list.c_str() + j + 1); j = list.find(',', j); }
                for (int c2 = a; c2 <= b && c2 < CPU_SETSIZE; c2++) { CPU_SET(c2, &set); n_set++; }
                i = j == std::string::npos ? list.size() : j + 1;
            }
        }
        cpu_set_t allowed;
        if (n_set > 0 && sched_getaffinity(0, sizeof allowed, &allowed) == 0) {
            n_set = 0;
            for (int c2 = 0; c2 < CPU_SETSIZE; c2++) {
                if (CPU_ISSET(c2, &set) && !CPU_ISSET(c2, &allowed)) CPU_CLR(c2, &set);
                if (CPU_ISSET(c2, &set)) n_set++;
            }
        }
        if (n_set > 0 && sched_setaffinity(0, sizeof set, &set) == 0) dev_node[k] = node;
    }
}

void Run::feed(size_t k)
{
    CpuScope cpu(CPU_FEEDER);
    const Api& L = *api;
    if (numa_bind) bind_to_node_of(k);
    if (L.create(&p, ctx_dev[k], &ctxs[k]) != TGSF_OK) die(L.last_error(nullptr));
    tgsf_ctx* fctx = ctxs[k];
    if (timing) (void)L.profile(fctx, 1);
    for (;;) {
        std::shared_ptr<Batch> b = to_gpu->get();
        if (!b) break;
        const double g0 = now_s();
        if (b->res.size() < b->recs.size()) b->res.resize(b->recs.size());
        const size_t fneed = (size_t)(b->bases / (uint64_t)std::max(p.min_len, 1)) + b->recs.size() + 16;
        if (b->frags.size() < fneed) b->frags.resize(fneed);
        const uint8_t* btext = reinterpret_cast<const uint8_t*>(b->base);
        tgsf_batch_in bi;
        memset(&bi, 0, sizeof bi);
        bi.seq = btext; bi.qual = btext;
        bi.offsets = b->off.data(); bi.qual_offsets = b->qoff.data(); bi.lengths = b->len.data();
        bi.n_reads = (uint32_t)b->recs.size(); bi.n_bytes = b->span;
        tgsf_batch_out bo{b->res.data(), b->frags.data(), (uint32_t)b->frags.size(), 0};
        if (L.submit(fctx, &bi, &bo) != TGSF_OK) die(L.last_error(fctx));
        { std::lock_guard<std::mutex> l(gpu_time_m); t_gpu += now_s() - g0; if (t_first == 0) t_first = now_s() - t_p0; }
        dev_submit_s[k] += now_s() - g0; dev_bytes[k] += b->span; dev_batches[k]++;
        b->n_frags = bo.n_frags;
        to_writer->put(std::move(b));
    }
    to_writer->put(nullptr);
}

void Run::batch_done(std::shared_ptr<Batch> b)
{
    if (b->out_bytes && release_output) mapped.release(b->dst, b->out_bytes);
    if (release_input) mapped.release(b->base, b->span);
    store.put(std::move(b));
}

void Run::filter_pass()
{
    to_gpu.reset(new Channel<std::shared_ptr<Batch>>(2 + ctxs.size()));
    to_writer.reset(new Channel<std::shared_ptr<Batch>>(256));
    if (!run_filter_pass) {
        RecordIndex::Cursor rd(*records_p);
        Rec r;
        while (rd.next(r)) {
            clean_recs.push_back({std::string_view(r.name, r.name_len), 1, r.seq, r.qual, r.len});
            clean_bases += r.len;
        }
    }

    std::thread reader([this] { reader_body(); });

    numa_bind = o.devices.size() > 1 || (link.world > 1 && ranks_own_gpus);
    if (const char* e = getenv("TGSF_NUMA")) numa_bind = atoi(e) > 0;
    dev_node.assign(ctx_dev.size(), -1);
    dev_submit_s.assign(ctx_dev.size(), 0.0);
    dev_bytes.assign(ctx_dev.size(), 0);
    dev_batches.assign(ctx_dev.size(), 0);
    std::vector<std::thread> feeders;
    for (size_t k = 0; k < ctxs.size(); k++) feeders.emplace_back([this, k] { feed(k); });

    fill_threads = std::max(1, std::min(o.n_thread, 16));
    fill_min = 1u << 20;
    if (const char* e = knob("TGSF_FILL_MIN_BYTES")) { const long long v = atoll(e); if (v > 0) fill_min = (uint64_t)v; }
    populate_threads = std::max(1, std::min(o.n_thread, 32));
    if (const char* e = knob("TGSF_POPULATE_THREADS")) { const int v = atoi(e); if (v >= 1 && v <= 64) populate_threads = v; }
    stride_bytes = streaming ? (128ull << 20) : (2ull << 30);
    if (const char* e = knob("TGSF_STRIDE_BYTES")) { const long long v = atoll(e); if (v > 0) stride_bytes = (uint64_t)v; }
    mapped.start_reserving(populate_threads, stride_bytes, (!streaming && text_size > (256u << 20)) ? (uint64_t)text_size / 4 : 0);
    {
        uint64_t early_min = 1ull << 30;
        if (const char* e = knob("TGSF_DOWN_EARLY_MIN")) early_min = strtoull(e, nullptr, 10);
        if (o.downsample && !streaming && in.mapped() && (uint64_t)text_size >= early_min) {
            uint64_t spec = (uint64_t)text_size / 4;
            if (o.genome_size > 0 && o.desired_depth > 0) spec = std::min<uint64_t>(spec, (2 * o.genome_size * (uint64_t)o.desired_depth) / (uint64_t)link.world + (uint64_t)text_size / 64);
            open_down_mapped(4 * (uint64_t)text_size + (1ull << 30), spec);
        }
    }
    const bool sync_exit = !detached();
    release_input = sync_exit && !streaming && in.mapped() && !o.downsample;
    release_output = sync_exit || streaming;
    mapped.start_filling(fill_threads, 16u << 20);
    std::thread writer([this] { writer_body(); });
    reader.join();
    for (std::thread& f : feeders) f.join();
    writer.join();
    mapped_out = mapped.is_open();
    mapped.finish();
    t_pipe = now_s() - t_p0;
}

}
```

### tgsfilter_amd/host/run_report.cpp

```cpp
#include "run.h"

#include <sys/stat.h>

namespace host {

std::vector<uint64_t> pack_rows(const std::vector<uint64_t>& v, int32_t bc2, uint32_t nb2)
{
    const size_t head = tgsf_ctr_bin_table(0, bc2, nb2);
    std::vector<uint64_t> out(v.begin(), v.begin() + (long)head);
    for (int b = 0; b < 4; b++) {
        const size_t at = tgsf_ctr_bin_table(b, bc2, nb2), n = (size_t)std::min<uint64_t>(v[TGSF_CTR_ROWS + (b >> 1)], nb2) * 5;
        out.insert(out.end(), v.begin() + (long)at, v.begin() + (long)(at + n));
    }
    return out;
}

void add_tallies(std::vector<uint64_t>& v, const std::vector<uint64_t>& part, int32_t bc2, uint32_t nb2)
{
    uint64_t rows[4];
    for (int q = 0; q < 4; q++) rows[q] = std::max(v[TGSF_CTR_ROWS + q], part[TGSF_CTR_ROWS + q]);
    const size_t head = tgsf_ctr_bin_table(0, bc2, nb2);
    for (size_t i = 0; i < head; i++) v[i] += part[i];
    for (int b = 0; b < 4; b++) {
        const size_t at = tgsf_ctr_bin_table(b, bc2, nb2), n = (size_t)std::min<uint64_t>(part[TGSF_CTR_ROWS + (b >> 1)], nb2) * 5;
        for (size_t i = 0; i < n; i++) v[at + i] += part[at + i];
    }
    for (int q = 0; q < 4; q++) v[TGSF_CTR_ROWS + q] = rows[q];
}

void add_rows(std::vector<uint64_t>& v, const std::vector<uint64_t>& ru, int32_t bc2, uint32_t nb2)
{
    const size_t head = tgsf_ctr_bin_table(0, bc2, nb2);
    if (ru.size() < head) die("a rank of the job sent a tally vector of another layout");
    std::vector<uint64_t> whole(v.size(), 0);
    std::copy(ru.begin(), ru.begin() + (long)head, whole.begin());
    size_t from = head;
    for (int b = 0; b < 4; b++) {
        const size_t at = tgsf_ctr_bin_table(b, bc2, nb2), n = (size_t)std::min<uint64_t>(ru[TGSF_CTR_ROWS + (b >> 1)], nb2) * 5;
        if (from + n > ru.size()) die("a rank of the job sent a tally vector of another layout");
        std::copy(ru.begin() + (long)from, ru.begin() + (long)(from + n), whole.begin() + (long)at);
        from += n;
    }
    add_tallies(v, whole, bc2, nb2);
}

static void add_context(const Api& L, tgsf_ctx* c, std::vector<uint64_t>& v, std::vector<uint64_t>& part, int32_t bc, uint32_t nbins)
{
    if (L.counters_used(c, part.data(), part.size(), nullptr) != TGSF_OK) die(L.last_error(c));
    add_tallies(v, part, bc, nbins);
}

void Run::sum_tallies()
{
    const Api& L = *api;
    tgsf_ctx* ctx = ctxs[0];
    void* rccl_comm = nullptr;
    int rccl_rc = TGSF_OK;
    std::string rccl_err;
    L.counters_len(ctx, &nw, &bc, &nbins);
    t.assign(nw, 0);
    std::vector<uint64_t> part(nw);
    t_x0 = now_s();
    own_raw_bases = raw_bases;
    const char* ex = getenv("TGSF_SHARD_EXCHANGE");
    const bool must_rccl = ex && !strcmp(ex, "rccl");
    for (tgsf_ctx* c : ctxs) add_context(L, c, t, part, bc, nbins);
    if (!sharded) return;

    if (use_rccl) {
        double rccl_patience = 120.0;
        if (const char* e = knob("TGSF_RCCL_INIT_TIMEOUT_S")) rccl_patience = atof(e);
        while (!rccl_state->done.load(std::memory_order_acquire) && now_s() - t_x0 < rccl_patience) usleep(2000);
        if (rccl_state->done.load(std::memory_order_acquire)) {
            rccl_up.join();
            rccl_rc = rccl_state->rc; rccl_err = rccl_state->err; rccl_comm = rccl_state->comm;
        } else {
            rccl_up.detach();
            rccl_rc = TGSF_E_HIP;
            rccl_err = "the communicator was not up " + std::to_string((int)rccl_patience) + " s after the filtering ended";
        }
        t_rccl_wait = now_s() - t_x0;
        if (link.max_u64(rccl_rc != TGSF_OK ? 1 : 0) != 0) {
            if (must_rccl) die("RCCL communicator: " + (rccl_err.empty() ? std::string("it failed on another rank") : rccl_err));
            if (rccl_rc != TGSF_OK) std::cerr << "Warning: rank " << link.rank << ": RCCL communicator: " << rccl_err << " -- the tallies are summed over the ranks' sockets" << std::endl;
            rccl_comm = nullptr;
            use_rccl = false;
        }
    }
    std::vector<uint64_t> reduced;
    if (use_rccl) {
        for (size_t k = 1; k < ctxs.size(); k++)
            if (L.counters_merge(ctxs[0], ctxs[k]) != TGSF_OK) die(L.last_error(ctxs[0]));
        struct Reduce { std::atomic<int> done{0}; int rc = TGSF_OK; std::string err; double s = 0; };
        const std::shared_ptr<Reduce> rd = std::make_shared<Reduce>();
        double patience = 60.0;
        if (const char* e = knob("TGSF_RCCL_ALLREDUCE_TIMEOUT_S")) patience = atof(e);
        const double a0 = now_s();
        std::thread helper([R = R, rd, c0 = ctxs[0], rccl_comm, rank = link.rank, world = link.world, a0] {
            if (const char* e = knob("TGSF_RCCL_ALLREDUCE_STALL_S")) usleep((useconds_t)(atof(e) * 1e6));
            rd->rc = R->allreduce_counters(c0, rccl_comm, rank, world, 0, nullptr);
            if (rd->rc != TGSF_OK) rd->err = R->last_error();
            rd->s = now_s() - a0;
            rd->done.store(1, std::memory_order_release);
        });
        while (!rd->done.load(std::memory_order_acquire) && now_s() - a0 < patience) usleep(500);
        int bad = 0;
        if (rd->done.load(std::memory_order_acquire)) {
            helper.join();
            t_allreduce = rd->s;
            if (rd->rc != TGSF_OK) { bad = 1; rccl_err = "tally all-reduce: " + rd->err; }
        } else {
            helper.detach();
            bad = 1;
            rccl_err = "the tally all-reduce had not returned after " + std::to_string((int)patience) + " s";
        }
        if (link.max_u64((uint64_t)bad) != 0) {
            if (must_rccl) die(rccl_err.empty() ? std::string("tally all-reduce: it failed on another rank") : rccl_err);
            if (bad) std::cerr << "Warning: rank " << link.rank << ": " << rccl_err << " -- the tallies summed over the ranks' sockets are used" << std::endl;
            use_rccl = false;
        } else {
            (void)R->comm_count(rccl_comm, &rccl_ranks);
            reduced.assign(nw, 0);
            add_context(L, ctxs[0], reduced, part, bc, nbins);
        }
    }
    BlobOut mine;
    mine.pod(raw_bases); mine.pod(clean_bases);
    mine.vec(raw_lens); mine.vec(clean_lens);
    mine.vec(pack_rows(t, bc, nbins));
    const std::vector<std::string> all = link.gather(mine.s);
    for (int k = 1; k < (int)all.size(); k++) {
        BlobIn in2(all[(size_t)k]);
        uint64_t rb = 0, cb = 0;
        std::vector<int> rl, cl;
        std::vector<uint64_t> ru;
        in2.pod(rb); in2.pod(cb); in2.vec(rl); in2.vec(cl); in2.vec(ru);
        raw_bases += rb; clean_bases += cb;
        const size_t r0 = raw_lens.size(), c0 = clean_lens.size();
        raw_lens.insert(raw_lens.end(), rl.begin(), rl.end());
        clean_lens.insert(clean_lens.end(), cl.begin(), cl.end());
        std::inplace_merge(raw_lens.begin(), raw_lens.begin() + (long)r0, raw_lens.end());
        if (!o.downsample) std::inplace_merge(clean_lens.begin(), clean_lens.begin() + (long)c0, clean_lens.end());
        add_rows(t, ru, bc, nbins);
    }
    tally_route = "summed on rank 0 over the ranks' sockets";
    if (use_rccl) {
        tally_route = "RCCL all-reduce on the devices";
        if (link.rank == 0) {
            if (pack_rows(reduced, bc, nbins) == pack_rows(t, bc, nbins)) { t.swap(reduced); tally_route += ", equal to the sum over the ranks' sockets"; }
            else {
                if (must_rccl) die("the all-reduced tally vector differs from the sum of the ranks' vectors over their sockets");
                std::cerr << "Warning: the all-reduced tally vector differs from the sum of the ranks' vectors over their sockets -- the sockets' sum is used" << std::endl;
                tally_route += " (DIFFERENT from the sum over the ranks' sockets, which is used)";
            }
        }
    }
    if (timing)
        fprintf(stderr, "SHARD %d/%d: bytes [%zu, %zu) of the text on device %d -> %s | tallies: %s (communicator ready after %.3f s of waiting, all-reduce %.4f s, %d ranks in it), exchange + gather %.3f s\n",
                link.rank, link.world, text_off, text_off + text_size, o.device, out_path.c_str(), tally_route.c_str(), t_rccl_wait, t_allreduce, rccl_ranks, now_s() - t_x0);
    if (use_rccl) R->comm_destroy(rccl_comm);
}

void Run::report()
{
    auto tables = [&](const std::vector<uint64_t>& v, bool clean) {
        SideTables s;
        s.bin_qual = &v[tgsf_ctr_bin_table(clean ? TGSF_B_CLEAN_QUAL : TGSF_B_RAW_QUAL, bc, nbins)];
        s.bin_cnt = &v[tgsf_ctr_bin_table(clean ? TGSF_B_CLEAN_CNT : TGSF_B_RAW_CNT, bc, nbins)];
        s.bin_rows = v[TGSF_CTR_ROWS + (clean ? 1 : 0)];
        s.q5 = &v[tgsf_ctr_end_table(clean ? TGSF_T_CLEAN5P_QUAL : TGSF_T_RAW5P_QUAL, bc)];
        s.c5 = &v[tgsf_ctr_end_table(clean ? TGSF_T_CLEAN5P_CNT : TGSF_T_RAW5P_CNT, bc)];
        s.q3 = &v[tgsf_ctr_end_table(clean ? TGSF_T_CLEAN3P_QUAL : TGSF_T_RAW3P_QUAL, bc)];
        s.c3 = &v[tgsf_ctr_end_table(clean ? TGSF_T_CLEAN3P_CNT : TGSF_T_RAW3P_CNT, bc)];
        s.end_rows = v[TGSF_CTR_ROWS + (clean ? 3 : 2)];
        s.diff_qual = &v[clean ? TGSF_CTR_CLEAN_DIFFQ : TGSF_CTR_RAW_DIFFQ];
        return s;
    };
    SideStats raw, clean;
    const int clean_num = (int)clean_lens.size();
    if (run_filter_pass && reports()) {
        if (raw_lens.empty()) die("no reads in the input");
        std::sort(raw_lens.begin(), raw_lens.end());
        side_stats(bc, raw_lens, raw_bases, tables(t, false), raw);
        if (!o.only_qc && !o.downsample) {
            if (clean_lens.empty()) die("no reads passed the filters");
            std::sort(clean_lens.begin(), clean_lens.end());
            side_stats(bc, clean_lens, clean_bases, tables(t, true), clean);
        }
        const uint64_t* d = &t[TGSF_CTR_DROPINFO];
        std::cerr << "INFO: " << raw_lens.size() << " reads with a total of " << raw_bases << " bases were input." << std::endl;
        if (!o.only_qc) {
            std::cerr << "INFO: " << d[0] << " reads were discarded with " << d[1] << " bases due to low quality." << std::endl;
            std::cerr << "INFO: " << d[2] << " reads have adapter at 5', 3' and middle." << std::endl;
            std::cerr << "INFO: " << d[3] << " reads have adapter at 5' and middle." << std::endl;
            std::cerr << "INFO: " << d[4] << " reads have adapter at 3' and middle." << std::endl;
            std::cerr << "INFO: " << d[5] << " reads have adapter at 5' and 3' end." << std::endl;
            std::cerr << "INFO: " << d[6] << " reads only have adapter at middle." << std::endl;
            std::cerr << "INFO: " << d[7] << " reads only have adapter at 5' end." << std::endl;
            std::cerr << "INFO: " << d[8] << " reads only have adapter at 3' end." << std::endl;
            std::cerr << "INFO: " << d[9] << " reads didn't have any adapter." << std::endl;
            std::cerr << "INFO: " << d[10] << " bases were trimmed due to the adapter or base content bias." << std::endl;
            std::cerr << "INFO: " << d[11] << " reads were discarded with " << d[12] << " bases due to the short length." << std::endl;
            std::cerr << "INFO: " << d[13] << " reads were discarded with " << d[14] << " bases due to low quality after split." << std::endl;
            if (o.min_repeat > 0)
                std::cerr << "INFO: " << d[15] << " reads were discarded with " << d[16] << " bases due to short repeat length." << std::endl;
            std::cerr << "INFO: " << clean_num << " reads with a total of " << clean_bases << " bases after filtering." << std::endl;
            if (!o.downsample && !o.out_file.empty()) {
                if (!sharded) std::cerr << "INFO: Filtered reads were written to: " << o.out_file << "." << std::endl;
                else std::cerr << "INFO: Filtered reads were written to: " << o.out_file << ".part0 ... " << o.out_file << ".part" << link.world - 1
                               << " (" << link.world << " parts; concatenated in this order they are the reads in input order)." << std::endl;
            }
        }
    }
    if (reports() && sharded && !o.out_file.empty() && !o.only_qc && !o.only_adapters) {
        const std::string list = o.out_file + ".parts";
        std::vector<std::string> earlier;
        {
            std::ifstream f(list);
            std::string line;
            if (f && std::getline(f, line) && line == "# tgsfilter parts, in order")
                while (std::getline(f, line)) if (!line.empty()) earlier.push_back(line);
        }
        std::vector<std::string> mine;
        for (int k = 0; k < link.world; k++) mine.push_back(o.out_file + ".part" + std::to_string(k));
        for (const std::string& e : earlier) {
            if (std::find(mine.begin(), mine.end(), e) != mine.end()) continue;
            const std::string stem = o.out_file + ".part";
            if (e.compare(0, stem.size(), stem) != 0 || e.size() == stem.size() || e.find_first_not_of("0123456789", stem.size()) != std::string::npos) continue;
            struct stat st;
            if (lstat(e.c_str(), &st) == 0 && S_ISREG(st.st_mode) && unlink(e.c_str()) == 0)
                std::cerr << "Warning: " << e << ", a part of an earlier job with more ranks, was removed." << std::endl;
        }
        for (int k = link.world; k < link.world + 1024; k++) {
            const std::string other = o.out_file + ".part" + std::to_string(k);
            struct stat st;
            if (lstat(other.c_str(), &st) != 0) { if (k >= link.world + 64) break; else continue; }
            std::cerr << "Warning: " << other << " exists and is not a part of this job (nor of an earlier one this tool listed): `cat " << o.out_file
                      << ".part*` would take it in -- the parts of this job are listed in " << list << "." << std::endl;
        }
        std::ofstream f(list, std::ios::trunc);
        f << "# tgsfilter parts, in order\n";
        for (const std::string& m : mine) f << m << "\n";
    }
    if (o.downsample && reports()) {
        if (down_lens.empty()) die("no reads to downsample");
        std::sort(down_lens.begin(), down_lens.end());
        side_stats(bc, down_lens, down_bases, tables(down_t, false), clean);
        clean.tab[8] = limit_decimals(std::round(clean.mean_qual * 1000) / 1000.0, 2);
        if (!o.filter)
            std::cerr << "INFO: " << (sharded ? down_job_recs : clean_recs.size()) << " reads with a total of " << (sharded ? down_job_bases : clean_bases) << " bases were input." << std::endl;
        std::cerr << "INFO: " << down_lens.size() << " reads with a total of " << down_bases << " bases after downsampling." << std::endl;
        if (!o.out_file.empty()) {
            if (!sharded) std::cerr << "INFO: Downsampled reads were written to: " << o.out_file << "." << std::endl;
            else std::cerr << "INFO: Downsampled reads were written to: " << o.out_file << ".part0 ... " << o.out_file << ".part" << link.world - 1
                           << " (" << link.world << " parts; concatenated in this order they are the reads in input order)." << std::endl;
        }
    }
    std::string qc = fasta_in ? "0" : "1";
    qc += o.only_qc ? "0" : ((!o.filter && o.downsample) ? "1" : "2");
    if (reports()) {
        std::ofstream ofs(html);
        write_report(ofs, qc, raw, clean);
        ofs.close();
        std::cerr << "INFO: Quality control report was written to: " << html << "." << std::endl;
    }
}

void Run::timing_lines()
{
    const Api& L = *api;
    if (timing) {
        Pool& fills = mapped.pool();
        const double t_busy = fills.busy_s();
        fprintf(stderr, "POOL: %zu jobs, busy %.3f, freeing job state %.3f, longest job %.3f, first job at %.3f, last job done at %.3f (pipeline start = 0, planner done at %.3f)\n",
                fills.jobs_, t_busy, fills.destroy_, fills.longest_, fills.first_ - t_p0, fills.last_ - t_p0, mapped.t_planned - t_p0);
        fprintf(stderr, "TIMING: total %.3f s | index+prepass %.3f | waiting for the library %.3f (load %.3f + device %.3f, beside the pre-pass) | "
                        "pipeline %.3f (batching %.3f, tgsf_submit summed over %zu feeders %.3f, plan+write %.3f, planner waiting %.3f, "
                        "first batch filtered after %.3f, fill tail %.3f, closing the output %.3f; stages overlap) | stats+report %.3f | %s (fallocate %.3f, mapping the reserved pages %.3f, fill threads busy %.3f summed)\n",
                now_s() - t_start, t_prepass, t_libwait, t_load, t_dev, t_pipe, t_parse, ctxs.size(), t_gpu, t_write, t_widle, t_first,
                mapped.t_fill_tail, mapped.t_close, now_s() - t_p0 - t_pipe, mapped_out ? "output: fallocate + mapped fill" : "output: writev", mapped.sink.t_falloc, mapped.t_populate_wait(), t_busy);
        fprintf(stderr, "RESERVE: planner waited %.3f s for pages of the output file\n", mapped.t_claim_wait);
    }
    if (timing) {
        float tot[TGSF_N_STAGES] = {0};
        uint32_t nb = 0;
        for (tgsf_ctx* c : ctxs) {
            float ms[TGSF_N_STAGES]; uint32_t n1 = 0;
            if (c && L.stage_times(c, ms, &n1) == TGSF_OK) { nb += n1; for (int i = 0; i < TGSF_N_STAGES; i++) tot[i] += ms[i]; }
        }
        double sum = 0;
        for (int i = 0; i < TGSF_N_STAGES; i++) sum += tot[i];
        char piece[256];
        snprintf(piece, sizeof piece, "GPU: kernels %.3f s summed over %zu contexts and %u batches (upper bound of the busy time: contexts overlap) = %.4f of the run |", sum * 1e-3, ctxs.size(), nb,
                 sum * 1e-3 / std::max(1e-9, now_s() - t_start));
        std::string line = piece;
        for (int i = 0; i < TGSF_N_STAGES; i++) if (tot[i] > 0) { snprintf(piece, sizeof piece, " %s %.1f ms", L.stage_name(i), tot[i]); line += piece; }
        line += "\n";
        fputs(line.c_str(), stderr);
    }
    if (timing) {
        for (size_t di = 0; di < o.devices.size(); di++) {
            if (std::find(o.devices.begin(), o.devices.begin() + (long)di, o.devices[di]) != o.devices.begin() + (long)di) continue;
            double sub = 0; uint64_t by = 0, nb2 = 0; int nf2 = 0, node = -1;
            for (size_t k = 0; k < ctx_dev.size(); k++)
                if (ctx_dev[k] == o.devices[di]) { sub += dev_submit_s[k]; by += dev_bytes[k]; nb2 += dev_batches[k]; nf2++; node = std::max(node, dev_node[k]); }
            fprintf(stderr, "DEVICE %d: %llu batches, %.2f GB of text through %d feeders, tgsf_submit %.3f s summed = %.1f GB/s per feeder, %.1f GB/s for the device over the pipeline's %.3f s%s\n",
                    o.devices[di], (unsigned long long)nb2, by * 1e-9, nf2, sub, sub > 0 ? by * 1e-9 / sub : 0.0, t_pipe > 0 ? by * 1e-9 / t_pipe : 0.0, t_pipe,
                    node >= 0 ? (" (feeders bound to NUMA node " + std::to_string(node) + ")").c_str() : "");
        }
    }
    if (timing) {
        const double proc = process_cpu_s();
        double own = 0;
        std::string line;
        char piece[160];
        for (int s = 0; s < CPU_N; s++) {
            double v = (double)cpu_ns()[s].load() * 1e-9;
            if (s == CPU_MAIN) v += (double)thread_cpu_ns() * 1e-9 - (double)cpu_ns()[CPU_PREPASS].load() * 1e-9;
            own += v;
            if (v >= 0.0005) { snprintf(piece, sizeof piece, "%s %s %.3f", line.empty() ? "" : ",", cpu_stage_name(s), v); line += piece; }
        }
        snprintf(piece, sizeof piece, "CPU: %.3f s of CPU time (user + system) for %.3f Gbases = %.4f CPU-s per Gbase |", proc, (double)own_raw_bases * 1e-9,
                 own_raw_bases ? proc / ((double)own_raw_bases * 1e-9) : 0.0);
        std::string head = piece;
        snprintf(piece, sizeof piece, " | threads of the runtime and others %.3f\n", proc - own);
        fputs((head + line + piece).c_str(), stderr);
    }
    if (timing && o.downsample)
        fprintf(stderr, "DOWN: selection %.3f | QC pass over the kept reads (%s, %.2f GB of them in %.2f GB of text): context %.3f, batches + submits %.3f (its own thread; %d submits %.3f, the first %.3f) | writing them %.3f (%s) | closing the output %.3f\n",
                t_dsel, d_in_place ? "read in place" : "packed", d_kept * 1e-9, d_span * 1e-9, t_dcreate, t_dqc, n_dsubmit, t_dsubmit, t_dfirst, t_dwrite, d_mapped ? "fallocate + threads into a mapping" : "writev", t_dclose);
    if (timing) {
        struct timespec ts; clock_gettime(CLOCK_REALTIME, &ts);
        fprintf(stderr, "CLOCK: main entered at %.6f, leaving at %.6f (epoch seconds)\n", t_epoch0, (double)ts.tv_sec + ts.tv_nsec * 1e-9);
    }
}

}
```

### tgsfilter_amd/host/run_second_pass.cpp

```cpp
#include "record_out.h"
#include "run.h"

namespace host {

void Run::second_pass(const std::vector<char>& keep)
{
    tgsf_ctx *qctx = nullptr, *qctx2 = nullptr;
    std::thread qc_pass = start_qc_feed(keep, qctx, qctx2);
    write_kept(keep);
    qc_pass.join();
    merge_down_tallies(qctx, qctx2);
}

std::thread Run::start_qc_feed(const std::vector<char>& keep, tgsf_ctx*& qctx, tgsf_ctx*& qctx2)
{
    tgsf_params qp = p;
    qp.filter = 0; qp.only_qc = 1; qp.n_adapters = 0; qp.min_repeat = 0;
    const bool down_no_qual = fasta_in || (run_filter_pass && !fastq_out);
    qp.no_qual = down_no_qual ? 1 : 0;
    qp.max_batch_bases = (1ull << 30); qp.max_batch_reads = 1u << 16;
    if (const char* e = knob("TGSF_DOWN_BATCH_BYTES")) { const long long v = atoll(e); if (v > (1 << 20) + 65536) qp.max_batch_bases = (uint64_t)v; }
    std::vector<uint32_t> by_addr;
    uint64_t kept_bytes = 0, kept_span = 0;
    for (size_t i = 0; i < clean_recs.size(); i++) {
        if (!keep[i]) continue;
        by_addr.push_back((uint32_t)i);
        kept_bytes += (down_no_qual ? 1u : 2u) * (uint64_t)clean_recs[i].len;
    }
    std::sort(by_addr.begin(), by_addr.end(), [&](uint32_t x, uint32_t y) { return clean_recs[x].seq < clean_recs[y].seq; });
    if (!by_addr.empty()) {
        const CleanRec& a = clean_recs[by_addr.front()];
        const CleanRec& z = clean_recs[by_addr.back()];
        kept_span = (uint64_t)((down_no_qual ? z.seq : std::max(z.seq, z.qual)) + z.len - a.seq);
        for (uint32_t i : by_addr) if (!down_no_qual && clean_recs[i].qual < clean_recs[i].seq) kept_span = 0;
    }
    const char* force = knob("TGSF_DOWN_QC");
    const bool in_place = kept_span > 0 && (force ? !strcmp(force, "text") : kept_bytes * 12 >= kept_span);
    d_in_place = in_place; d_kept = (double)kept_bytes; d_span = (double)kept_span;
    const size_t room = (size_t)std::min<uint64_t>(qp.max_batch_bases, kept_bytes / (down_no_qual ? 1 : 2) + 16 * by_addr.size() + 128);
    return std::thread([this, &keep, &qctx, &qctx2, qp, in_place, kept_span, room, by_addr = std::move(by_addr)] {
        CpuScope cpu(CPU_DOWNSAMPLE);
        const double q0 = now_s();
        if (api->create(&qp, o.devices[0], &qctx) != TGSF_OK) die(api->last_error(nullptr));
        t_dcreate = now_s() - q0;
        if (in_place) feed_in_place(by_addr, qp, kept_span, qctx, qctx2);
        else feed_packed(keep, qp, room, qctx);
        t_dqc = now_s() - q0 - t_dcreate;
    });
}

void Run::feed_in_place(const std::vector<uint32_t>& by_addr, const tgsf_params& qp, uint64_t kept_span, tgsf_ctx* qctx, tgsf_ctx*& qctx2)
{
    const Api& L = *api;
    const bool down_no_qual = qp.no_qual != 0;
    struct TextBatch { const char* base = nullptr; uint64_t span = 0; std::vector<uint64_t> off, qoff; std::vector<uint32_t> len; };
    int workers = kept_span >= (2ull << 30) ? 2 : 1;
    if (const char* e = knob("TGSF_DOWN_FEEDERS")) workers = atoi(e) >= 2 ? 2 : 1;
    Channel<std::shared_ptr<TextBatch>> todo(2);
    std::mutex tm;
    auto work = [&](tgsf_ctx* c) {
        std::vector<tgsf_read_result> res;
        std::vector<tgsf_fragment> fr(16);
        for (;;) {
            std::shared_ptr<TextBatch> tb = todo.get();
            if (!tb) break;
            res.resize(tb->len.size());
            tgsf_batch_in bi; memset(&bi, 0, sizeof bi);
            bi.seq = bi.qual = reinterpret_cast<const uint8_t*>(tb->base);
            bi.offsets = tb->off.data(); bi.qual_offsets = tb->qoff.data(); bi.lengths = tb->len.data();
            bi.n_reads = (uint32_t)tb->len.size(); bi.n_bytes = tb->span;
            tgsf_batch_out bo{res.data(), fr.data(), (uint32_t)fr.size(), 0};
            const double s0 = now_s();
            if (L.submit(c, &bi, &bo) != TGSF_OK) die(L.last_error(c));
            std::lock_guard<std::mutex> l(tm);
            t_dsubmit += now_s() - s0; if (!n_dsubmit++) t_dfirst = now_s() - s0;
        }
    };
    std::thread second;
    if (workers == 2) second = std::thread([&] {
        CpuScope cpu2(CPU_DOWNSAMPLE);
        if (L.create(&qp, o.devices[0], &qctx2) != TGSF_OK) die(L.last_error(nullptr));
        work(qctx2);
    });
    std::thread first([&] { CpuScope cpu2(CPU_DOWNSAMPLE); work(qctx); });
    std::shared_ptr<TextBatch> tb(new TextBatch);
    auto flush_text = [&] {
        if (tb->len.empty()) return;
        todo.put(std::move(tb));
        tb.reset(new TextBatch);
    };
    for (uint32_t i : by_addr) {
        const CleanRec& c = clean_recs[i];
        const char* e = down_no_qual ? c.seq + c.len : c.qual + c.len;
        if (tb->base && ((uint64_t)(e - tb->base) > qp.max_batch_bases - (1u << 20) || tb->len.size() >= qp.max_batch_reads)) flush_text();
        if (!tb->base) tb->base = c.seq;
        tb->off.push_back((uint64_t)(c.seq - tb->base));
        tb->qoff.push_back((uint64_t)((down_no_qual ? c.seq : c.qual) - tb->base));
        tb->len.push_back(c.len);
        tb->span = std::max(tb->span, (uint64_t)(e - tb->base));
        if (tb->span > qp.max_batch_bases) die("record larger than a batch");
    }
    flush_text();
    for (int k = 0; k < workers; k++) todo.put(nullptr);
    first.join();
    if (second.joinable()) second.join();
}

void Run::feed_packed(const std::vector<char>& keep, const tgsf_params& qp, size_t room, tgsf_ctx* qctx)
{
    const Api& L = *api;
    const bool down_no_qual = qp.no_qual != 0;
    std::vector<uint8_t> bs, bq; std::vector<uint64_t> boff; std::vector<uint32_t> blen;
    std::vector<tgsf_read_result> bres; std::vector<tgsf_fragment> bfr(16);
    auto run = [&] {
        if (blen.empty()) return;
        bres.resize(blen.size());
        bs.resize(bs.size() + 64); bq.resize(bq.size() + 64);
        tgsf_batch_in bi; memset(&bi, 0, sizeof bi);
        bi.seq = bs.data(); bi.qual = bq.data(); bi.offsets = boff.data(); bi.lengths = blen.data();
        bi.n_reads = (uint32_t)blen.size(); bi.n_bytes = bs.size() - 64;
        tgsf_batch_out bo{bres.data(), bfr.data(), (uint32_t)bfr.size(), 0};
        const double s0 = now_s();
        if (L.submit(qctx, &bi, &bo) != TGSF_OK) die(L.last_error(qctx));
        t_dsubmit += now_s() - s0; if (!n_dsubmit++) t_dfirst = now_s() - s0;
        bs.clear(); bq.clear(); boff.clear(); blen.clear();
    };
    bs.reserve(room); bq.reserve(room);
    for (size_t i = 0; i < clean_recs.size(); i++) {
        if (!keep[i]) continue;
        const CleanRec& c = clean_recs[i];
        if (bs.size() + c.len > qp.max_batch_bases - (1u << 20) || blen.size() >= qp.max_batch_reads) run();
        const size_t o0 = (bs.size() + 15) & ~size_t(15);
        bs.resize(o0); bq.resize(o0);
        bs.insert(bs.end(), c.seq, c.seq + c.len);
        if (!down_no_qual) bq.insert(bq.end(), c.qual, c.qual + c.len); else bq.resize(bs.size());
        boff.push_back(o0); blen.push_back(c.len);
    }
    run();
}

void Run::write_kept(const std::vector<char>& keep)
{
    const double w0 = now_s();
    const char* mn = knob("TGSF_DOWN_MAP_MIN");
    const uint64_t map_min = mn ? strtoull(mn, nullptr, 10) : (256ull << 20);
    std::vector<uint32_t> kept;
    std::vector<uint64_t> at;
    uint64_t total_out = 0;
    if (plain_file_out()) {
        for (size_t i = 0; i < clean_recs.size(); i++) {
            if (!keep[i]) continue;
            kept.push_back((uint32_t)i); at.push_back(total_out);
            total_out += record_bytes(clean_recs[i], fastq_out);
        }
    }
    if (!down_mapped.is_open() && total_out >= std::max<uint64_t>(map_min, 1)) open_down_mapped(total_out, 0);
    d_mapped = down_mapped.is_open();
    if (d_mapped) {
        const uint64_t piece = std::max<uint64_t>(1, std::min<uint64_t>(64ull << 20, stride_bytes / 4 + 1));
        down_mapped.start_filling(fill_threads, piece);
        size_t r0 = 0;
        while (r0 < kept.size()) {
            size_t r1 = (size_t)(std::lower_bound(at.begin() + (long)r0, at.end(), at[r0] + piece) - at.begin());
            if (r1 <= r0) r1 = r0 + 1;
            const uint64_t bytes = (r1 < at.size() ? at[r1] : total_out) - at[r0];
            char* const dst = down_mapped.claim(bytes, total_out);
            down_mapped.fill([this, &kept, r0, r1, dst, bytes] {
                fill_records(dst, dst + bytes, r0, r1, fastq_out, [&](size_t r) -> const CleanRec& { return clean_recs[kept[r]]; });
                if (release_output) down_mapped.release(dst, bytes);
            });
            r0 = r1;
        }
        down_mapped.finish();
    } else {
        std::string name;
        for (size_t i = 0; i < clean_recs.size(); i++)
            if (keep[i]) gather_record(out, clean_recs[i], fastq_out, name);
    }
    t_dwrite = now_s() - w0;
}

void Run::merge_down_tallies(tgsf_ctx* qctx, tgsf_ctx* qctx2)
{
    const Api& L = *api;
    uint64_t qnw = 0; int32_t qbc = 0; uint32_t qnb = 0;
    L.counters_len(qctx, &qnw, &qbc, &qnb);
    down_t.resize(qnw);
    if (L.counters(qctx, down_t.data(), qnw) != TGSF_OK) die(L.last_error(qctx));
    L.destroy(qctx);
    if (qctx2) {
        std::vector<uint64_t> t2(qnw);
        if (L.counters(qctx2, t2.data(), qnw) != TGSF_OK) die(L.last_error(qctx2));
        L.destroy(qctx2);
        add_tallies(down_t, t2, qbc, qnb);
    }
    if (sharded) {
        BlobOut mine;
        mine.vec(pack_rows(down_t, qbc, qnb));
        const std::vector<std::string> all = link.gather(mine.s);
        for (int k = 1; k < (int)all.size(); k++) {
            BlobIn in2(all[(size_t)k]);
            std::vector<uint64_t> ru;
            in2.vec(ru);
            add_rows(down_t, ru, qbc, qnb);
        }
    }
}

}
```

Measured before the change: 4.845.

## Plan device buffers into slab allocations, pin staging in one block, reuse prepass context

Device buffers and adapter tables are no longer allocated one by one. They are now recorded in a plan and committed together, possibly as a single slab. The pinned status word and the two staging buffers share one host allocation. The alignment workspace is grown and reused across calls instead of being malloc'd and freed each time, and the prepass adapter search reuses one library context for both ends instead of creating two. The aim is to cut context-creation and allocation overhead on the host, at the cost of more complex ownership (the pool is now owned separately) and new timing instrumentation.

```diff
diff --git a/tgsfilter_amd/csrc/tgsf_emul_rt.h b/tgsfilter_amd/csrc/tgsf_emul_rt.h
--- a/tgsfilter_amd/csrc/tgsf_emul_rt.h
+++ b/tgsfilter_amd/csrc/tgsf_emul_rt.h
@@ -5,7 +5,9 @@
 static int rt_set_device(int) { return 0; }
 static int rt_malloc(void** p, size_t n) { *p = calloc(n ? n : 1, 1); return *p ? 0 : 1; }
 static void rt_free(void* p) { free(p); }
+static int rt_host_malloc(void** p, size_t) { *p = nullptr; return 1; }
 static void rt_host_free(void*) {}
+constexpr bool kRtOneBlock = false;
 static int rt_memset(void* p, int v, size_t n, rt_stream) { memset(p, v, n); return 0; }
 static int rt_h2d(void* d, const void* s, size_t n, rt_stream) { memcpy(d, s, n); return 0; }
 static int rt_d2h(void* d, const void* s, size_t n, rt_stream) { memcpy(d, s, n); return 0; }
diff --git a/tgsfilter_amd/csrc/tgsf_lib.hip b/tgsfilter_amd/csrc/tgsf_lib.hip
--- a/tgsfilter_amd/csrc/tgsf_lib.hip
+++ b/tgsfilter_amd/csrc/tgsf_lib.hip
@@ -51,6 +51,7 @@
     rt_event ev_fork, ev_join;
     uint32_t* h_pinned = nullptr;
     static constexpr size_t kStageBytes = 32u << 20;
+    size_t stage_bytes = kStageBytes;
     uint8_t* stage[2] = {nullptr, nullptr};
     rt_event stage_ev[2] = {nullptr, nullptr};
     uint32_t h_words_[8];
@@ -64,6 +65,10 @@
     uint32_t* bp_ring = nullptr;
     uint32_t h_ovf[TGSF_MAX_ENQUEUED];
     uint32_t pool_regrown = 0;
+    void* pool_own = nullptr;
+    size_t pool_own_bytes = 0;
+    dev_space align_ws;
+    dev_tally tally;
 };
 
 static const int kMaxLenParam = 1 << 28;
@@ -108,12 +113,21 @@
     }
 }
 
-static int build_tables(tgsf_ctx* c)
-{
-    DevParams& P = c->P;
+struct Tables {
+    std::vector<uint8_t> ad;
+    std::vector<uint64_t> fwd, rev, top, fwd_w, rev_w;
+    uint8_t* d_ad = nullptr;
+    uint64_t *d_f = nullptr, *d_r = nullptr, *d_t = nullptr, *d_fw = nullptr, *d_rw = nullptr;
+};
+
+static void plan_tables(tgsf_ctx* c, Tables& T, dev_plan& pl)
+{
+    const DevParams& P = c->P;
     const int A = c->params.n_adapters;
-    std::vector<uint8_t> ad((size_t)kMaxAdapters * kMaxQ, 0);
-    std::vector<uint64_t> fwd, rev, top((size_t)kMaxAdapters * 256, 0);
+    std::vector<uint8_t>& ad = T.ad;
+    std::vector<uint64_t>&fwd = T.fwd, &rev = T.rev, &top = T.top;
+    ad.assign((size_t)kMaxAdapters * kMaxQ, 0);
+    top.assign((size_t)kMaxAdapters * 256, 0);
     fill_peq(c->adapters, kMaxAdapters, kPeqW, fwd, rev);
     for (int a = 0; a < A; a++) {
         const int Q = P.Q[a];
@@ -125,30 +139,33 @@
                 top[(size_t)a * 256 + sym] = (fwd[((size_t)a * 256 + sym) * kPeqW] << sh) | pad;
         }
     }
-    uint8_t* d_ad; uint64_t *d_f, *d_r, *d_t;
-    int e;
-    if ((e = dev_alloc(c, &d_ad, ad.size()))) return e;
-    if ((e = dev_alloc(c, &d_f, fwd.size()))) return e;
-    if ((e = dev_alloc(c, &d_r, rev.size()))) return e;
-    if ((e = dev_alloc(c, &d_t, top.size()))) return e;
-    rt_h2d(d_ad, ad.data(), ad.size(), c->stream);
-    rt_h2d(d_f, fwd.data(), fwd.size() * 8, c->stream);
-    rt_h2d(d_r, rev.data(), rev.size() * 8, c->stream);
-    rt_h2d(d_t, top.data(), top.size() * 8, c->stream);
+    pl.add(&T.d_ad, ad.size());
+    pl.add(&T.d_f, fwd.size());
+    pl.add(&T.d_r, rev.size());
+    pl.add(&T.d_t, top.size());
+    if (P.max_nw > 4) {
+        fill_peq(c->adapters, (size_t)A, kWideNW, T.fwd_w, T.rev_w);
+        pl.add(&T.d_fw, T.fwd_w.size());
+        pl.add(&T.d_rw, T.rev_w.size());
+    }
+}
+
+static void upload_tables(tgsf_ctx* c, const Tables& T)
+{
+    DevParams& P = c->P;
+    rt_h2d(T.d_ad, T.ad.data(), T.ad.size(), c->stream);
+    rt_h2d(T.d_f, T.fwd.data(), T.fwd.size() * 8, c->stream);
+    rt_h2d(T.d_r, T.rev.data(), T.rev.size() * 8, c->stream);
+    rt_h2d(T.d_t, T.top.data(), T.top.size() * 8, c->stream);
     rt_sync(c->stream);
-    P.adapter = d_ad; P.peq_fwd = d_f; P.peq_rev = d_r; P.peq_top = d_t;
+    P.adapter = T.d_ad; P.peq_fwd = T.d_f; P.peq_rev = T.d_r; P.peq_top = T.d_t;
     P.peq_fwd_w = P.peq_rev_w = nullptr;
     if (P.max_nw > 4) {
-        fill_peq(c->adapters, (size_t)A, kWideNW, fwd, rev);
-        uint64_t *d_fw, *d_rw;
-        if ((e = dev_alloc(c, &d_fw, fwd.size()))) return e;
-        if ((e = dev_alloc(c, &d_rw, rev.size()))) return e;
-        rt_h2d(d_fw, fwd.data(), fwd.size() * 8, c->stream);
-        rt_h2d(d_rw, rev.data(), rev.size() * 8, c->stream);
+        rt_h2d(T.d_fw, T.fwd_w.data(), T.fwd_w.size() * 8, c->stream);
+        rt_h2d(T.d_rw, T.rev_w.data(), T.rev_w.size() * 8, c->stream);
         rt_sync(c->stream);
-        P.peq_fwd_w = d_fw; P.peq_rev_w = d_rw;
-    }
-    return 0;
+        P.peq_fwd_w = T.d_fw; P.peq_rev_w = T.d_rw;
+    }
 }
 
 extern "C" int tgsf_abi_version(void) { return TGSF_ABI_VERSION; }
@@ -259,15 +276,21 @@
         for (rt_event e : c->ev[k]) rt_event_destroy(e);
         for (rt_event e : c->ev_aux[k]) rt_event_destroy(e);
     }
+    if (knob("TGSF_TRACE_ALLOC")) {
+        const dev_tally& t = c->tally;
+        fprintf(stderr, "tgsf: context memory: %u device allocations of %zu bytes holding %u arrays; %u pinned allocations of %zu bytes; "
+                        "candidate pool regrown %u times; alignment workspace grown %u times to %zu bytes\n",
+                t.blocks + (c->pool_own ? 1u : 0u) + (unsigned)c->align_ws.parts.size(), t.block_bytes + c->pool_own_bytes + c->align_ws.bytes, t.arrays,
+                t.pinned, t.pinned_bytes, c->pool_regrown, t.fits_grown, c->align_ws.bytes);
+    }
     if (c->h_pinned) rt_host_free(c->h_pinned);
-    for (int i = 0; i < 2; i++) {
-        if (c->stage[i]) rt_host_free(c->stage[i]);
-        rt_event_destroy(c->stage_ev[i]);
-    }
+    for (int i = 0; i < 2; i++) rt_event_destroy(c->stage_ev[i]);
     rt_event_destroy(c->ev_fork);
     rt_event_destroy(c->ev_join);
     if (c->aux) rt_stream_destroy(c->aux);
     if (c->own_stream && c->stream) rt_stream_destroy(c->stream);
+    dev_space_free(c->align_ws);
+    if (c->pool_own) rt_free(c->pool_own);
     dev_free_all(c);
     delete c;
 }
@@ -398,11 +421,19 @@
     if ((he = hipSetDevice(c->device)) != hipSuccess) return fail(nullptr, TGSF_E_HIP, "hipSetDevice: %s", hipGetErrorString(he));
     if ((he = hipStreamCreateWithFlags(&c->stream, hipStreamNonBlocking)) != hipSuccess) return fail(nullptr, TGSF_E_HIP, "hipStreamCreate: %s", hipGetErrorString(he));
     c->own_stream = true;
+    const bool staged = c->params.max_batch_bases > (8u << 20);
+    if (const char* e = knob("TGSF_STAGE_BYTES")) { const long long v = atoll(e); if (v >= 65536 && v <= (1ll << 30)) c->stage_bytes = (size_t)v; }
+    const size_t pin_sizes[3] = {64, c->stage_bytes, c->stage_bytes};
+    size_t pin_off[3], pin_total = 0;
+    (void)slab_layout(pin_sizes, staged ? 3 : 1, 0, pin_off, &pin_total);
+    if (!staged) pin_total = 64;
     uint32_t* pw = nullptr;
-    if (hipHostMalloc((void**)&pw, 64, hipHostMallocDefault) == hipSuccess && pw) {
+    if (rt_host_malloc((void**)&pw, pin_total) == 0 && pw) {
         memset(pw, 0, 64);
         c->h_pinned = pw; c->h_status = pw; c->pend_nf_p = pw + 4;
-    }
+        c->tally.pinned = 1; c->tally.pinned_bytes = pin_total;
+    } else if (staged)
+        return fail(nullptr, TGSF_E_HIP, "pinned staging buffers: allocation failed");
     int lo = 0, hi = 0;
     (void)hipDeviceGetStreamPriorityRange(&lo, &hi);
     he = hipStreamCreateWithPriority(&c->aux, hipStreamNonBlocking, hi);
@@ -410,87 +441,90 @@
         (he = hipEventCreateWithFlags(&c->ev_fork, hipEventDisableTiming)) != hipSuccess ||
         (he = hipEventCreateWithFlags(&c->ev_join, hipEventDisableTiming)) != hipSuccess)
         return fail(nullptr, TGSF_E_HIP, "auxiliary stream: %s", hipGetErrorString(he));
-    if (c->params.max_batch_bases > (8u << 20)) {
-        for (int i = 0; i < 2; i++)
-            if (hipHostMalloc((void**)&c->stage[i], tgsf_ctx::kStageBytes, hipHostMallocDefault) != hipSuccess ||
-                hipEventCreateWithFlags(&c->stage_ev[i], hipEventDisableTiming) != hipSuccess)
+    if (staged)
+        for (int i = 0; i < 2; i++) {
+            c->stage[i] = (uint8_t*)c->h_pinned + pin_off[1 + i];
+            if (hipEventCreateWithFlags(&c->stage_ev[i], hipEventDisableTiming) != hipSuccess)
                 return fail(nullptr, TGSF_E_HIP, "pinned staging buffers: allocation failed");
-    }
+        }
 #endif
     c->last_stream = c->stream;
     return TGSF_OK;
 }
 
-static int allocate(tgsf_ctx* c, const Sizing& S)
+static void plan_buffers(tgsf_ctx* c, const Sizing& S, dev_plan& pl)
 {
     DevBatch& B = c->B;
     const size_t n = c->cap_reads;
     const int A = std::max(c->params.n_adapters, 1);
     const size_t tiles = 2 * ((size_t)B.max_tiles + 2);
-    int e = 0;
-    if (!e) e = dev_alloc(c, &c->d_seq, S.cap_bytes);
-    if (!e) e = dev_alloc(c, &c->d_qual, S.cap_bytes);
-    if (!e) e = dev_alloc(c, &c->d_off, n + 1);
-    if (!e) e = dev_alloc(c, &c->d_qoff, n + 1);
-    if (!e) e = dev_alloc(c, &c->d_lenin, n);
-    if (!e) e = dev_alloc(c, &B.len, n);
-    if (!e) e = dev_alloc(c, &B.sumq, n);
-    if (!e) e = dev_alloc(c, &B.flags, n);
-    if (!e) e = dev_alloc(c, &B.clip5, n * A);
-    if (!e) e = dev_alloc(c, &B.clip3, n * A);
-    if (!e) e = dev_alloc(c, &B.mid_head, n);
-    if (!e) e = dev_alloc(c, &B.mid_best, n * A);
-    if (!e) e = dev_alloc(c, &B.mid_cnt, n);
-    if (!e) e = dev_alloc(c, &B.mid_gate, n * A);
-    if (!e) e = dev_alloc(c, &B.pool, (size_t)B.pool_cap);
-    if (!e) e = dev_alloc(c, &B.pool_n, 4);
-    if (!e) e = dev_alloc(c, &B.seg_cnt, n + 1);
-    if (!e) e = dev_alloc(c, &B.chk_cnt, n + 1);
+    pl.add(&c->d_seq, S.cap_bytes);
+    pl.add(&c->d_qual, S.cap_bytes);
+    pl.add(&c->d_off, n + 1);
+    pl.add(&c->d_qoff, n + 1);
+    pl.add(&c->d_lenin, n);
+    pl.add(&B.len, n);
+    pl.add(&B.sumq, n);
+    pl.add(&B.flags, n);
+    pl.add(&B.clip5, n * A);
+    pl.add(&B.clip3, n * A);
+    pl.add(&B.mid_head, n);
+    pl.add(&B.mid_best, n * A);
+    pl.add(&B.mid_cnt, n);
+    pl.add(&B.mid_gate, n * A);
+    pl.add(&B.pool, (size_t)B.pool_cap);
+    pl.add(&B.pool_n, 4);
+    pl.add(&B.seg_cnt, n + 1);
+    pl.add(&B.chk_cnt, n + 1);
     if (c->suffix_filter) {
-        if (!e) e = dev_alloc(c, &B.chk_mark, (size_t)4 * (size_t)(S.cap_chunks / 32u + 8u));
-        if (!e) e = dev_alloc(c, &B.rc_list, (size_t)B.rc_cap + 1);
-        if (!e) e = dev_alloc(c, &B.rc_n, 4);
-    }
-    if (!e) e = dev_alloc(c, &B.nfr, n + 1);
-    if (!e) e = dev_alloc(c, &B.scan_part, n / kScanTile + 2);
-    if (!e) e = dev_alloc(c, &B.trimmed, n);
-    if (!e) e = dev_alloc(c, &B.rep_next, 2 + (size_t)B.rep_long_cap);
+        pl.add(&B.chk_mark, (size_t)4 * (size_t)(S.cap_chunks / 32u + 8u));
+        pl.add(&B.rc_list, (size_t)B.rc_cap + 1);
+        pl.add(&B.rc_n, 4);
+    }
+    pl.add(&B.nfr, n + 1);
+    pl.add(&B.scan_part, n / kScanTile + 2);
+    pl.add(&B.trimmed, n);
+    pl.add(&B.rep_next, 2 + (size_t)B.rep_long_cap);
     if (B.rep_tab_log2) {
-        if (!e) e = dev_alloc(c, &B.rep_tab, (size_t)1 << B.rep_tab_log2);
-        if (!e) e = dev_alloc(c, &B.rep_lock, 4);
-        if (!e) rt_memset(B.rep_lock, 0, 16, c->stream);
-    }
-    if (!e) e = dev_alloc(c, &B.tile_hist, tiles);
-    if (!e) e = dev_alloc(c, &B.tile_cnt, tiles);
-    if (!e) e = dev_alloc(c, &B.tile_base, tiles);
-    if (!e) e = dev_alloc(c, &B.tile_fill, tiles);
-    if (!e) e = dev_alloc(c, &B.seg_info, 4);
-    if (!e) e = dev_alloc(c, &B.perm, S.nitems);
-    if (!e) e = dev_alloc(c, &B.work, 2 * (size_t)B.work_cap);
-    if (!e) e = dev_alloc(c, &B.frag_off, (size_t)B.fcap);
-    if (!e) e = dev_alloc(c, &B.frag_qoff, (size_t)B.fcap);
-    if (!e) e = dev_alloc(c, &B.frag_len, (size_t)B.fcap);
-    if (!e) e = dev_alloc(c, &B.frag_sum, (size_t)B.fcap);
-    if (!e) e = dev_alloc(c, &B.frag_read, (size_t)B.fcap);
-    if (!e) e = dev_alloc(c, &B.frag_start, (size_t)B.fcap);
-    if (!e) e = dev_alloc(c, &B.frag_flags, (size_t)B.fcap);
-    if (!e) e = dev_alloc(c, &B.raw_tab, 2 * (size_t)c->n_bins * 5);
-    if (!e) e = dev_alloc(c, &B.whole, n);
-    if (!e) e = dev_alloc(c, &B.plan, 4);
+        pl.add(&B.rep_tab, (size_t)1 << B.rep_tab_log2);
+        pl.add(&B.rep_lock, 4);
+    }
+    pl.add(&B.tile_hist, tiles);
+    pl.add(&B.tile_cnt, tiles);
+    pl.add(&B.tile_base, tiles);
+    pl.add(&B.tile_fill, tiles);
+    pl.add(&B.seg_info, 4);
+    pl.add(&B.perm, S.nitems);
+    pl.add(&B.work, 2 * (size_t)B.work_cap);
+    pl.add(&B.frag_off, (size_t)B.fcap);
+    pl.add(&B.frag_qoff, (size_t)B.fcap);
+    pl.add(&B.frag_len, (size_t)B.fcap);
+    pl.add(&B.frag_sum, (size_t)B.fcap);
+    pl.add(&B.frag_read, (size_t)B.fcap);
+    pl.add(&B.frag_start, (size_t)B.fcap);
+    pl.add(&B.frag_flags, (size_t)B.fcap);
+    pl.add(&B.raw_tab, 2 * (size_t)c->n_bins * 5);
+    pl.add(&B.whole, n);
+    pl.add(&B.plan, 4);
     if (B.bp_allowed) {
-        if (!e) e = dev_alloc(c, &B.spec, n);
-        if (!e) e = dev_alloc(c, &B.spec_sum, n);
-        if (!e) e = dev_alloc(c, &B.bp_state, 4);
-        if (!e) e = dev_alloc(c, &c->bp_ring, TGSF_MAX_ENQUEUED);
-    }
-    if (!e) e = dev_alloc(c, &B.scratch, S.scratch_waves * B.scratch_wave_words);
-    if (!e) e = dev_alloc(c, &B.ctr, (size_t)c->ctr_words);
-    if (!e) e = dev_alloc(c, &B.status, 4);
-    if (!e) e = dev_alloc(c, &c->ovf_ring, TGSF_MAX_ENQUEUED);
-    if (!e) e = dev_alloc(c, &c->d_out_reads, n);
-    if (!e) e = dev_alloc(c, &c->d_out_frags, (size_t)B.fcap);
-    if (!e) e = dev_alloc(c, &c->d_out_nfrags, 4);
-    if (e) return e;
+        pl.add(&B.spec, n);
+        pl.add(&B.spec_sum, n);
+        pl.add(&B.bp_state, 4);
+        pl.add(&c->bp_ring, TGSF_MAX_ENQUEUED);
+    }
+    pl.add(&B.scratch, S.scratch_waves * B.scratch_wave_words);
+    pl.add(&B.ctr, (size_t)c->ctr_words);
+    pl.add(&B.status, 4);
+    pl.add(&c->ovf_ring, TGSF_MAX_ENQUEUED);
+    pl.add(&c->d_out_reads, n);
+    pl.add(&c->d_out_frags, (size_t)B.fcap);
+    pl.add(&c->d_out_nfrags, 4);
+}
+
+static int init_buffers(tgsf_ctx* c)
+{
+    DevBatch& B = c->B;
+    if (B.rep_tab_log2) rt_memset(B.rep_lock, 0, 16, c->stream);
     rt_memset(B.ctr, 0, c->ctr_words * 8, c->stream);
     rt_memset(B.status, 0, 16, c->stream);
     rt_memset(c->ovf_ring, 0, TGSF_MAX_ENQUEUED * 4, c->stream);
@@ -539,7 +573,17 @@
     c->B = S.B; c->cap_chunks = S.cap_chunks; c->scratch_cols = S.scratch_cols; P.seg_cols = S.seg_cols;
     c->flat_scan = S.flat_scan; c->suffix_filter = S.suffix_filter; c->no_hot32 = S.no_hot32;
 
-    if ((e = bring_up(c)) || (e = build_tables(c)) || (e = allocate(c, S))) {
+    Tables T;
+    dev_plan pl;
+    if (!(e = bring_up(c))) {
+        plan_tables(c, T, pl);
+        plan_buffers(c, S, pl);
+        if (!(e = dev_commit(c, pl, c->tally))) {
+            upload_tables(c, T);
+            e = init_buffers(c);
+        }
+    }
+    if (e) {
         if (!c->error.empty()) g_create_error = c->error;
         tgsf_destroy(c);
         return e;
@@ -772,8 +816,8 @@
                 rc = fail(c, TGSF_E_CAPACITY, "middle-adapter candidates: no device memory for %llu slots (%.1f GB)", (unsigned long long)want, (double)want * sizeof(MidCand) * 1e-9);
                 break;
             }
-            for (void*& q : c->allocs) if (q == (void*)c->B.pool) q = np;
-            rt_free(c->B.pool);
+            if (c->pool_own) rt_free(c->pool_own);
+            c->pool_own = np; c->pool_own_bytes = (size_t)want * sizeof(MidCand) + 64;
             c->B.pool = (MidCand*)np; c->B.pool_cap = (uint32_t)want;
             B.pool = c->B.pool; B.pool_cap = c->B.pool_cap;
             c->pool_regrown++;
@@ -923,8 +967,8 @@
     (void)hipGetLastError();
     if (!known && c->stage[0] && n > (1u << 20)) {
         int he = 0, k = 0;
-        for (uint64_t o = 0; o < n; o += tgsf_ctx::kStageBytes, k ^= 1) {
-            const size_t m = (size_t)std::min<uint64_t>(tgsf_ctx::kStageBytes, n - o);
+        for (uint64_t o = 0; o < n; o += c->stage_bytes, k ^= 1) {
+            const size_t m = (size_t)std::min<uint64_t>(c->stage_bytes, n - o);
             (void)hipEventSynchronize(c->stage_ev[k]);
             memcpy(c->stage[k], src + o, m);
             he |= (int)hipMemcpyAsync(dst + o, c->stage[k], m, hipMemcpyHostToDevice, st);
@@ -1203,14 +1247,15 @@
     (void)rt_set_device(c->device);
     uint8_t *d_seq = nullptr, *d_aid = nullptr; uint64_t* d_off = nullptr; uint32_t* d_len = nullptr;
     int32_t *d_k = nullptr, *d_res = nullptr, *d_ends = nullptr;
-    int e = 0;
-    e |= rt_malloc((void**)&d_seq, n_bytes + 16);
-    e |= rt_malloc((void**)&d_aid, n);
-    e |= rt_malloc((void**)&d_off, (size_t)n * 8);
-    e |= rt_malloc((void**)&d_len, (size_t)n * 4);
-    e |= rt_malloc((void**)&d_k, (size_t)n * 4);
-    e |= rt_malloc((void**)&d_res, (size_t)n * 16);
-    e |= rt_malloc((void**)&d_ends, (size_t)n * 8);
+    dev_plan pl;
+    pl.add(&d_seq, (size_t)n_bytes);
+    pl.add(&d_aid, (size_t)n);
+    pl.add(&d_off, (size_t)n);
+    pl.add(&d_len, (size_t)n);
+    pl.add(&d_k, (size_t)n);
+    pl.add(&d_res, (size_t)n * 4);
+    pl.add(&d_ends, (size_t)n * 2);
+    int e = dev_fit(c->align_ws, pl, c->alloc_slack, c->tally);
     rt_stream st = c->stream;
     if (!e) {
         e |= rt_h2d(d_seq, seq, n_bytes, st);
@@ -1228,6 +1273,5 @@
         e |= rt_d2h(ends, d_ends, (size_t)n * 8, st);
         e |= rt_sync(st);
     }
-    rt_free(d_seq); rt_free(d_aid); rt_free(d_off); rt_free(d_len); rt_free(d_k); rt_free(d_res); rt_free(d_ends);
     return e ? fail(c, TGSF_E_HIP, "tgsf_align_windows: device operation failed") : TGSF_OK;
 }
diff --git a/tgsfilter_amd/csrc/tgsf_rt.h b/tgsfilter_amd/csrc/tgsf_rt.h
--- a/tgsfilter_amd/csrc/tgsf_rt.h
+++ b/tgsfilter_amd/csrc/tgsf_rt.h
@@ -18,7 +18,9 @@
 static int rt_set_device(int device) { return (int)hipSetDevice(device); }
 static int rt_malloc(void** p, size_t n) { return (int)hipMalloc(p, n ? n : 1); }
 static void rt_free(void* p) { (void)hipFree(p); }
+static int rt_host_malloc(void** p, size_t n) { return (int)hipHostMalloc(p, n, hipHostMallocDefault); }
 static void rt_host_free(void* p) { (void)hipHostFree(p); }
+constexpr bool kRtOneBlock = true;
 static int rt_memset(void* p, int v, size_t n, rt_stream s) { return (int)hipMemsetAsync(p, v, n, s); }
 static int rt_h2d(void* d, const void* s, size_t n, rt_stream st) { return (int)hipMemcpyAsync(d, s, n, hipMemcpyHostToDevice, st); }
 static int rt_d2h(void* d, const void* s, size_t n, rt_stream st) { return (int)hipMemcpyAsync(d, s, n, hipMemcpyDeviceToHost, st); }
@@ -71,3 +73,89 @@
 }
 
 static void dev_free_all(rt_ctx* c) { for (void* p : c->allocs) rt_free(p); }
+
+constexpr size_t kSlabAlign = 4096;
+static bool slab_layout(const size_t* bytes, size_t n, size_t slack, size_t* off, size_t* total)
+{
+    size_t at = 0;
+    for (size_t i = 0; i < n; i++) {
+        off[i] = at;
+        size_t share = bytes[i] ? bytes[i] : 1;
+        if (share > SIZE_MAX - slack || share + slack > SIZE_MAX - (kSlabAlign - 1)) return false;
+        share = (share + slack + kSlabAlign - 1) & ~(kSlabAlign - 1);
+        if (share > SIZE_MAX - at) return false;
+        at += share;
+    }
+    *total = at;
+    return true;
+}
+
+struct dev_plan {
+    struct item { void** pp; size_t bytes; };
+    std::vector<item> items;
+    bool overflow = false;
+    template <class T>
+    void add(T** p, size_t count)
+    {
+        if (count > SIZE_MAX / sizeof(T)) overflow = true;
+        items.push_back({(void**)p, count * sizeof(T)});
+    }
+    bool lay_out(size_t slack, std::vector<size_t>& off, size_t* total) const
+    {
+        std::vector<size_t> bytes(items.size());
+        for (size_t i = 0; i < items.size(); i++) bytes[i] = items[i].bytes;
+        off.resize(items.size());
+        return !overflow && slab_layout(bytes.data(), bytes.size(), slack, off.data(), total);
+    }
+};
+
+struct dev_tally { uint32_t blocks = 0, arrays = 0, pinned = 0, fits_grown = 0; size_t block_bytes = 0, pinned_bytes = 0; };
+
+static int dev_commit(rt_ctx* c, const dev_plan& pl, dev_tally& t)
+{
+    std::vector<size_t> off;
+    size_t total = 0;
+    if (!pl.lay_out(c->alloc_slack, off, &total))
+        return fail(c, TGSF_E_HIP, "device allocation of %zu arrays failed: their sizes do not fit 64 bits", pl.items.size());
+    int e = 0;
+    if (kRtOneBlock) {
+        void* base = nullptr;
+        if ((e = rt_malloc(&base, total))) return fail(c, TGSF_E_HIP, "device allocation of %zu bytes failed: %s", total, rt_errstr(e));
+        c->allocs.push_back(base);
+        for (size_t i = 0; i < pl.items.size(); i++) *pl.items[i].pp = (char*)base + off[i];
+    } else
+        for (const dev_plan::item& it : pl.items) {
+            void* v = nullptr;
+            if ((e = rt_malloc(&v, it.bytes + c->alloc_slack))) return fail(c, TGSF_E_HIP, "device allocation of %zu bytes failed: %s", total, rt_errstr(e));
+            c->allocs.push_back(v);
+            *it.pp = v;
+        }
+    t.blocks += kRtOneBlock ? 1u : (uint32_t)pl.items.size(); t.block_bytes += total; t.arrays += (uint32_t)pl.items.size();
+    return 0;
+}
+
+struct dev_space { std::vector<void*> parts; size_t bytes = 0; };
+static void dev_space_free(dev_space& w) { for (void* p : w.parts) rt_free(p); w.parts.clear(); }
+static int dev_fit(dev_space& w, const dev_plan& pl, size_t slack, dev_tally& t)
+{
+    std::vector<size_t> off;
+    size_t total = 0;
+    if (!pl.lay_out(slack, off, &total)) return TGSF_E_HIP;
+    const bool grow = total > w.bytes;
+    if (grow || !kRtOneBlock) {
+        dev_space_free(w);
+        if (kRtOneBlock) {
+            void* base = nullptr;
+            if (rt_malloc(&base, total)) { w.bytes = 0; return TGSF_E_HIP; }
+            w.parts.push_back(base);
+        } else
+            for (const dev_plan::item& it : pl.items) {
+                void* v = nullptr;
+                if (rt_malloc(&v, it.bytes + slack)) { w.bytes = 0; return TGSF_E_HIP; }
+                w.parts.push_back(v);
+            }
+        if (grow) { w.bytes = total; t.fits_grown++; }
+    }
+    for (size_t i = 0; i < pl.items.size(); i++) *pl.items[i].pp = kRtOneBlock ? (void*)((char*)w.parts[0] + off[i]) : w.parts[i];
+    return 0;
+}
diff --git a/tgsfilter_amd/host/prepass.cpp b/tgsfilter_amd/host/prepass.cpp
--- a/tgsfilter_amd/host/prepass.cpp
+++ b/tgsfilter_amd/host/prepass.cpp
@@ -86,22 +86,28 @@
 }
 
 static double pp_now() { return std::chrono::duration<double>(std::chrono::steady_clock::now().time_since_epoch()).count(); }
-static double g_pp_create = 0, g_pp_align = 0; static int g_pp_calls = 0;
-
-static void adapter_search(const Options& o, const std::vector<std::string>& ends, std::string& adapter, float& depth)
-{
-    adapter.clear(); depth = 0.f;
-    float min_sim = o.mid_sim;
+static double g_pp_create = 0, g_pp_align = 0, g_pp_destroy = 0; static int g_pp_calls = 0;
+
+struct SearchContext {
+    tgsf_ctx* ctx = nullptr;
+    int k[22];
+    float min_sim = 0.9f;
+    size_t per_call = 4096;
+    void create(const Options& o);
+    void destroy();
+};
+
+void SearchContext::create(const Options& o)
+{
+    min_sim = o.mid_sim;
     if (min_sim < 0.9) min_sim = 0.9f;
-    if (ends.empty()) return;
-
+    if (const char* e = knob("TGSF_PREPASS_CALL")) { const long long v = atoll(e); if (v >= 1 && v <= 15360) per_call = (size_t)v; }
     tgsf_params p;
     memset(&p, 0, sizeof p);
     p.struct_size = sizeof p;
     p.min_len = 100; p.max_len = 2147483647; p.min_q = 0; p.max_q = 255; p.bc_len = 0;
     p.end_len = 0; p.extra_len = 0; p.end_sim = 0.75f; p.mid_sim = 0.9f; p.filter = 1; p.qtype = 33;
     p.n_adapters = 22;
-    int k[22];
     size_t max_q = 0;
     for (int a = 0; a < 22; a++) {
         p.adapters[a] = kAdapterLib[a];
@@ -110,14 +116,31 @@
         max_q = std::max(max_q, (size_t)p.adapter_len[a]);
     }
     p.end_match_len = 2; p.mid_match_len = (int)max_q;
-    const size_t per_call = 4096;
     p.max_batch_reads = (uint32_t)(per_call * 22 / (22 * 2) + 64);
     p.max_batch_bases = 1 << 20; p.max_read_len = 1 << 16;
-    tgsf_ctx* ctx = nullptr;
     const double c0 = pp_now();
     if (lib().create(&p, o.devices.empty() ? o.device : o.devices[0], &ctx) != TGSF_OK) { std::cerr << "Error: " << lib().last_error(nullptr) << std::endl; quit(255); }
-
     g_pp_create += pp_now() - c0;
+}
+
+void SearchContext::destroy()
+{
+    if (!ctx) return;
+    const double d0 = pp_now();
+    lib().destroy(ctx);
+    g_pp_destroy += pp_now() - d0;
+    ctx = nullptr;
+}
+
+static void adapter_search(const Options& o, SearchContext& sc, const std::vector<std::string>& ends, std::string& adapter, float& depth)
+{
+    adapter.clear(); depth = 0.f;
+    if (ends.empty()) return;
+    if (!sc.ctx) sc.create(o);
+    tgsf_ctx* const ctx = sc.ctx;
+    const int* const k = sc.k;
+    const float min_sim = sc.min_sim;
+    const size_t per_call = sc.per_call;
     std::unordered_map<int, int> maps;
     std::vector<uint8_t> buf; std::vector<uint64_t> off; std::vector<uint32_t> len; std::vector<uint8_t> aid;
     std::vector<int32_t> kk, res, eds;
@@ -142,7 +165,6 @@
             if (res[(size_t)i * 4 + 1] > 0)
                 maps[(int)aid[i]] += res[(size_t)i * 4 + 2] - res[(size_t)i * 4 + 0];
     }
-    lib().destroy(ctx);
     std::vector<std::pair<int, int>> vec(maps.begin(), maps.end());
     std::sort(vec.begin(), vec.end(), [](const std::pair<int, int>& a, const std::pair<int, int>& b) { return a.second > b.second; });
     if (vec.empty()) return;
@@ -209,8 +231,11 @@
         if (o.head_trim < 0 && o.tail_trim < 0 && R.trim5p > o.bc_len) R.trim5p = o.bc_len;
         t_bc = pp_now() - t1;
         if (o.adapter_file.empty()) {
-            adapter_search(o, ends5, R.adapter5p, R.depth5p);
-            adapter_search(o, ends3, R.adapter3p, R.depth3p);
+            SearchContext sc;
+            adapter_search(o, sc, ends5, R.adapter5p, R.depth5p);
+            adapter_search(o, sc, ends3, R.adapter3p, R.depth3p);
+            sc.destroy();
+            R.t_destroy = g_pp_destroy;
         }
     }
     if (getenv("TGSF_TIMING"))
diff --git a/tgsfilter_amd/host/prepass.h b/tgsfilter_amd/host/prepass.h
--- a/tgsfilter_amd/host/prepass.h
+++ b/tgsfilter_amd/host/prepass.h
@@ -17,6 +17,7 @@
     int trim5p = 0, trim3p = 0;
     std::string adapter5p, adapter3p;
     float depth5p = 0.f, depth3p = 0.f;
+    double t_destroy = 0;
 };
 
 PrepassResult run_prepass(Options& o, const std::function<bool(Rec&)>& next_record);
diff --git a/tgsfilter_amd/host/run.h b/tgsfilter_amd/host/run.h
--- a/tgsfilter_amd/host/run.h
+++ b/tgsfilter_amd/host/run.h
@@ -35,6 +35,8 @@
     bool timing = false;
     double t_epoch0 = 0, t_start = 0;
     double t_prepass = 0, t_pipe = 0, t_parse = 0, t_gpu = 0, t_write = 0, t_widle = 0, t_first = 0;
+    double t_destroy = 0;
+    double t_create = 0;
 
     std::string html;
     bool fasta_in = false;
diff --git a/tgsfilter_amd/host/run_pipeline.cpp b/tgsfilter_amd/host/run_pipeline.cpp
--- a/tgsfilter_amd/host/run_pipeline.cpp
+++ b/tgsfilter_amd/host/run_pipeline.cpp
@@ -119,7 +119,9 @@
     CpuScope cpu(CPU_FEEDER);
     const Api& L = *api;
     if (numa_bind) bind_to_node_of(k);
+    const double c0 = now_s();
     if (L.create(&p, ctx_dev[k], &ctxs[k]) != TGSF_OK) die(L.last_error(nullptr));
+    { std::lock_guard<std::mutex> l(gpu_time_m); t_create = std::max(t_create, now_s() - c0); }
     tgsf_ctx* fctx = ctxs[k];
     if (timing) (void)L.profile(fctx, 1);
     for (;;) {
diff --git a/tgsfilter_amd/host/run_report.cpp b/tgsfilter_amd/host/run_report.cpp
--- a/tgsfilter_amd/host/run_report.cpp
+++ b/tgsfilter_amd/host/run_report.cpp
@@ -276,9 +276,9 @@
                 fills.jobs_, t_busy, fills.destroy_, fills.longest_, fills.first_ - t_p0, fills.last_ - t_p0, mapped.t_planned - t_p0);
         fprintf(stderr, "TIMING: total %.3f s | index+prepass %.3f | waiting for the library %.3f (load %.3f + device %.3f, beside the pre-pass) | "
                         "pipeline %.3f (batching %.3f, tgsf_submit summed over %zu feeders %.3f, plan+write %.3f, planner waiting %.3f, "
-                        "first batch filtered after %.3f, fill tail %.3f, closing the output %.3f; stages overlap) | stats+report %.3f | %s (fallocate %.3f, mapping the reserved pages %.3f, fill threads busy %.3f summed)\n",
+                        "first batch filtered after %.3f, longest tgsf_create %.3f, tgsf_destroy %.3f, fill tail %.3f, closing the output %.3f; stages overlap) | stats+report %.3f | %s (fallocate %.3f, mapping the reserved pages %.3f, fill threads busy %.3f summed)\n",
                 now_s() - t_start, t_prepass, t_libwait, t_load, t_dev, t_pipe, t_parse, ctxs.size(), t_gpu, t_write, t_widle, t_first,
-                mapped.t_fill_tail, mapped.t_close, now_s() - t_p0 - t_pipe, mapped_out ? "output: fallocate + mapped fill" : "output: writev", mapped.sink.t_falloc, mapped.t_populate_wait(), t_busy);
+                t_create, t_destroy + pp.t_destroy, mapped.t_fill_tail, mapped.t_close, now_s() - t_p0 - t_pipe, mapped_out ? "output: fallocate + mapped fill" : "output: writev", mapped.sink.t_falloc, mapped.t_populate_wait(), t_busy);
         fprintf(stderr, "RESERVE: planner waited %.3f s for pages of the output file\n", mapped.t_claim_wait);
     }
     if (timing) {
diff --git a/tgsfilter_amd/host/run_second_pass.cpp b/tgsfilter_amd/host/run_second_pass.cpp
--- a/tgsfilter_amd/host/run_second_pass.cpp
+++ b/tgsfilter_amd/host/run_second_pass.cpp
@@ -187,11 +187,15 @@
     L.counters_len(qctx, &qnw, &qbc, &qnb);
     down_t.resize(qnw);
     if (L.counters(qctx, down_t.data(), qnw) != TGSF_OK) die(L.last_error(qctx));
+    const double d0 = now_s();
     L.destroy(qctx);
+    t_destroy += now_s() - d0;
     if (qctx2) {
         std::vector<uint64_t> t2(qnw);
         if (L.counters(qctx2, t2.data(), qnw) != TGSF_OK) die(L.last_error(qctx2));
+        const double d1 = now_s();
         L.destroy(qctx2);
+        t_destroy += now_s() - d1;
         add_tallies(down_t, t2, qbc, qnb);
     }
     if (sharded) {
```

Result: slower. 4.366 (-9.9%).
